# brendel-group/cl-ica

Hardware: AMD Instinct MI355X
Metric: training steps/sec (B=6144, n=10 MLP) (higher is better)
Workload: dtype f32 via f16x2 split (3 fp16 MFMA products of scaled two-piece operands, fp32 accumulate)

## Files before the change

cl_ica_amd/csrc/linear.hip:

```cpp
#include "common.h"
#include <string.h>
#include "wgrad_shared.h"
#include "split16.h"
#include "adam_math.h"
#include <stdlib.h>
#include <algorithm>

namespace clica {
bool skinny_fwd(const float* X, int64_t ldx, const float* W, int64_t ldw, const float* bias, float* Y, int64_t ldy,
                int64_t M, int64_t N, int64_t K, int leaky, float slope, hipStream_t st);
bool skinny_dgrad(const float* dY, int64_t lddy, const float* W, int64_t ldw, const float* Xact, int64_t ldxa, float slope,
                  float* dX, int64_t lddx, int64_t M, int64_t N, int64_t K, hipStream_t st);

namespace conv16 {
void launch_slab_sum(const float* slab1, int n1, float* out1, const float* slab2, int n2, float* out2, int splits, int accumulate, hipStream_t st);
}
namespace gemm {

typedef float f32x16 __attribute__((ext_vector_type(16)));

constexpr int BK = 32;
constexpr int RED_THREADS = 256;

enum Epi { EPI_BIAS_ACT = 0, EPI_DACT = 1, EPI_SLAB = 2 };
// ... 1045 lines not shown
        float* dst = G.dW[q] + i * G.lddw[q] + j;
        t.x = G.accumulate ? (*dst + t.x) : t.x;
        *dst = t.x;
        if (with_adam) adam_apply1(A, s_c, dst, t.x);
      }
    }
  } else {
    reduce_units<false>(G.dbslab[q], G.splits[q], M, (int64_t)(b - G.dw_blocks[q]) * 64, red, t, e);
    float* db = G.db[q];
    if (w == 0 && e < M) {
      t.x = G.accumulate ? (db[e] + t.x) : t.x;
      db[e] = t.x;
      if (with_adam) adam_apply1(A, s_c, db + e, t.x);
    }
  }
}

static void launch_slab_reduce(const float* slab, const float* dbslab, int splits, int64_t M, int64_t N, float* dW, int64_t lddw,
                               float* db, int accumulate, hipStream_t st) {
  const int64_t total = M * N;
  const bool v4 = (N % 4 == 0) && (lddw % 4 == 0) && ((reinterpret_cast<uintptr_t>(dW) & 15) == 0);
  const int dw_blocks = (int)ceil_div(v4 ? total / 4 : total, 64);
  const int db_blocks = db ? (int)ceil_div(M, 64) : 0;
  if (v4)
    hipLaunchKernelGGL(slab_reduce_k<true>, dim3((unsigned)(dw_blocks + db_blocks)), dim3(RED_THREADS), 0, st, slab, splits, M, N, dW, lddw,
                       dbslab, db, accumulate, dw_blocks);
  else
    hipLaunchKernelGGL(slab_reduce_k<false>, dim3((unsigned)(dw_blocks + db_blocks)), dim3(RED_THREADS), 0, st, slab, splits, M, N, dW, lddw,
                       dbslab, db, accumulate, dw_blocks);
}

static bool aligned16(const void* p) { return (reinterpret_cast<uintptr_t>(p) & 15) == 0; }

struct Cfg { int bm, bn, wm, wn; };
constexpr Cfg kCfgs[] = {
    {192, 128, 2, 4},
    {128, 128, 2, 4},
    {64, 128, 2, 2},
    {128, 128, 2, 2},
    {192, 64, 2, 2},
    {96, 128, 1, 4},
};
constexpr int kNumCfgs = sizeof(kCfgs) / sizeof(kCfgs[0]);

template <int BM, int BN, int WM, int WN, int STAGES, bool A_CONTIG, bool B_CONTIG, int EPI>
static int launch_cfg(const Args& g, int splits, hipStream_t st, const char* who) {
  constexpr int THREADS = 64 * WM * WN;
  const bool vec = aligned16(g.A) && aligned16(g.B) && (g.lda % 4 == 0) && (g.ldb % 4 == 0) &&
                   (A_CONTIG ? (g.Kc % 4 == 0) : (g.M % 4 == 0)) && (B_CONTIG ? (g.Kc % 4 == 0) : (g.N % 4 == 0));
  dim3 grid((unsigned)ceil_div(g.N, BN), (unsigned)ceil_div(g.M, BM), (unsigned)splits), block(THREADS);
  constexpr size_t lds = STAGES * (Tile<BM, A_CONTIG, THREADS>::LDS_FLOATS + Tile<BN, B_CONTIG, THREADS>::LDS_FLOATS) * sizeof(float);
  if (vec) {
    auto k = gemm_k<BM, BN, WM, WN, STAGES, A_CONTIG, B_CONTIG, EPI, true>;
    static bool once = ((void)hipFuncSetAttribute(reinterpret_cast<const void*>(k), hipFuncAttributeMaxDynamicSharedMemorySize, (int)lds), true);
    (void)once;
    hipLaunchKernelGGL(k, grid, block, lds, st, g);
  } else {
    auto k = gemm_k<BM, BN, WM, WN, STAGES, A_CONTIG, B_CONTIG, EPI, false>;
    static bool once = ((void)hipFuncSetAttribute(reinterpret_cast<const void*>(k), hipFuncAttributeMaxDynamicSharedMemorySize, (int)lds), true);
    (void)once;
    hipLaunchKernelGGL(k, grid, block, lds, st, g);
  }
  return launch_status(who);
}

template <bool A_CONTIG, bool B_CONTIG, int EPI>
static int launch(int cfg, const Args& g, int splits, hipStream_t st, const char* who) {
  switch (cfg) {
    case 0: return launch_cfg<192, 128, 2, 4, 3, A_CONTIG, B_CONTIG, EPI>(g, splits, st, who);
    case 1: return launch_cfg<128, 128, 2, 4, 3, A_CONTIG, B_CONTIG, EPI>(g, splits, st, who);
    case 2: return launch_cfg<64, 128, 2, 2, 2, A_CONTIG, B_CONTIG, EPI>(g, splits, st, who);
    case 4: return launch_cfg<192, 64, 2, 2, 2, A_CONTIG, B_CONTIG, EPI>(g, splits, st, who);
    case 5: return launch_cfg<96, 128, 1, 4, 2, A_CONTIG, B_CONTIG, EPI>(g, splits, st, who);
    default: return launch_cfg<128, 128, 2, 2, 2, A_CONTIG, B_CONTIG, EPI>(g, splits, st, who);
  }
}

struct Tuning { int cfg_fwd, cfg_dgrad, cfg_wgrad; bool skinny; };
static Tuning& tuning() { static Tuning t{-1, -1, -1, true}; return t; }
static bool use_skinny() { return tuning().skinny; }

static int cfg_fwd(int64_t N) {
  const int e = tuning().cfg_fwd;
  return (e >= 0 && e < kNumCfgs) ? e : ((N > 128) ? 5 : 2);
}
static int cfg_dgrad() {
  const int e = tuning().cfg_dgrad;
  return (e >= 0 && e < kNumCfgs) ? e : 2;
}

struct WgradPlan { int cfg, splits; int64_t k_per_split; };
static WgradPlan plan_wgrad(int64_t M , int64_t N , int64_t Kc) {
  WgradPlan p;
  p.cfg = (M > 128 && N > 128) ? 1 : 2;
  const int e = tuning().cfg_wgrad;
  if (e >= 0 && e < kNumCfgs) p.cfg = e;
  const Cfg c = kCfgs[p.cfg];
  const int64_t tiles = ceil_div(M, c.bm) * ceil_div(N, c.bn);
  int64_t want = kNumCU / tiles; if (want < 1) want = 1;
  const int64_t max_s = ceil_div(Kc, (int64_t)BK * 4);
  if (want > max_s) want = max_s;
  if (want < 1) want = 1;
  p.k_per_split = ceil_div(ceil_div(Kc, want), (int64_t)BK) * BK;
  p.splits = (int)ceil_div(Kc, p.k_per_split);
  return p;
}

struct GroupPlan { int splits; int64_t k_per_split; int tiles; int tiny_splits; int64_t tiny_kps; int n_tiny; };
constexpr int GBM = 128, GBN = 128;
static int group_kind(int32_t N, int32_t K) {
  if (tiny_eligible(N, K, TINY_THREADS)) return 2;
  if (N % 4 != 0 || K % 4 != 0) return 0;
  if (N > 128 || K > 128) return N >= K ? 3 : 4;
  return 1;
}
static void group_tile(int kind, int* bm, int* bn) {
  *bm = kind == 3 ? 256 : 128; *bn = kind == 4 ? 256 : 128;
}
static GroupPlan plan_wgrad_group(int64_t Mrows, int n, const int32_t* N, const int32_t* K) {
  GroupPlan p{};
  for (int l = 0; l < n; ++l) {
    const int kind = group_kind(N[l], K[l]);
    if (kind == 2) { ++p.n_tiny; continue; }
    int bm, bn; group_tile(kind, &bm, &bn);
    p.tiles += (int)(ceil_div(N[l], bm) * ceil_div(K[l], bn));
  }
  const int64_t max_s = std::max<int64_t>(1, std::min<int64_t>(64, ceil_div(Mrows, (int64_t)BK * 4)));
  double best = 1e300;
  p.splits = 1; p.k_per_split = ceil_div(Mrows, (int64_t)BK) * BK;
  for (int64_t s = 1; s <= max_s && p.tiles > 0; ++s) {
    const int64_t kps = ceil_div(ceil_div(Mrows, s), (int64_t)BK) * BK;
    const int64_t sp = ceil_div(Mrows, kps);
    const int64_t rounds = ceil_div((int64_t)p.tiles * sp, kNumCU);
    const double cost = (double)rounds * (kps + 32.0) + 8.0 * sp;
    if (cost < best) { best = cost; p.splits = (int)sp; p.k_per_split = kps; }
  }
  if (p.n_tiny > 0) wgrad_tiny_plan(Mrows, p.n_tiny, &p.tiny_splits, &p.tiny_kps);
  return p;
}
static bool group_is_tiny(const GroupPlan& p, int32_t N, int32_t K) { return p.n_tiny > 0 && group_kind(N, K) == 2; }
static size_t group_ws_layout(const GroupPlan& p, int n, const int32_t* N, const int32_t* K, size_t* slab_off, size_t* db_off) {
  size_t off = 0;
  for (int l = 0; l < n; ++l) {
    const size_t sp = group_is_tiny(p, N[l], K[l]) ? p.tiny_splits : p.splits;
    if (slab_off) slab_off[l] = off;
    off += align_up(sp * N[l] * K[l] * sizeof(float), 256);
    if (db_off) db_off[l] = off;
    off += align_up(sp * N[l] * sizeof(float), 256);
  }
  return off;
}


bool wgrad_tiny_shape(int32_t N, int32_t K) { return group_kind(N, K) == 2; }
void wgrad_tiny_plan(int64_t Mrows, int n_tiny, int* splits, int64_t* k_per_split) {
  int64_t ts = std::max<int64_t>(1, kNumCU / std::max(1, n_tiny));
  const int64_t cap = std::max<int64_t>(1, Mrows / (2 * TINY_ROWS));
  if (ts > cap) ts = cap;
  *k_per_split = ceil_div(ceil_div(Mrows, ts), (int64_t)TINY_ROWS) * TINY_ROWS;
  *splits = (int)ceil_div(Mrows, *k_per_split);
}
int launch_wgrad_tiny(const TinyArgs& T, int splits, hipStream_t st) {
  constexpr size_t tiny_lds = (size_t)(TINY_ROWS * TINY_MAX_LG + TINY_ROWS * TINY_MAX_S) * sizeof(float) + 1024;
  static bool once_t = ((void)hipFuncSetAttribute(reinterpret_cast<const void*>(wgrad_tiny_k), hipFuncAttributeMaxDynamicSharedMemorySize, (int)tiny_lds), true);
  (void)once_t;
  hipLaunchKernelGGL(wgrad_tiny_k, dim3((unsigned)splits, (unsigned)T.n), dim3(TINY_THREADS), tiny_lds, st, T);
  return launch_status("clica_mlp_wgrad(tiny)");
}
int launch_slab_reduce_group(const ReduceGroupArgs& R, int blocks, hipStream_t st) {
  const int front = (R.adam.p && R.adam.s16_state) ? s16::kS16UpdateBlocks : 0;
  hipLaunchKernelGGL(slab_reduce_group_k, dim3((unsigned)(blocks + front)), dim3(RED_THREADS), 0, st, R);
  return launch_status("clica_mlp_wgrad(reduce)");
}
int slab_reduce_entry(ReduceGroupArgs& R, int l, int first_block, int sp, const float* slab, const float* dbslab,
                      float* dW, int64_t lddw, float* db, int32_t N, int32_t K) {
  const bool v4 = (K % 4 == 0) && (lddw % 4 == 0) && aligned16(dW);
  R.vec4[l] = v4 ? 1 : 0; R.splits[l] = sp;
  R.dw_blocks[l] = (int)ceil_div(v4 ? (int64_t)N * K / 4 : (int64_t)N * K, reduce_flat(sp, v4) ? RED_THREADS : 64);
  R.first[l] = first_block;
  R.slab[l] = slab; R.dbslab[l] = dbslab; R.dW[l] = dW; R.db[l] = db;
  R.M[l] = N; R.N[l] = K; R.lddw[l] = lddw;
  return R.dw_blocks[l] + (db ? (int)ceil_div(N, 64) : 0);
}

}
}

using namespace clica;
using namespace clica::gemm;

extern "C" int clica_mlp_wgrad_workspace_bytes(int64_t M, int32_t n_layers, const int32_t* N, const int32_t* K, size_t* bytes) {
  CLICA_CHECK_ARG(bytes && N && K && M > 0 && n_layers >= 1 && n_layers <= MAXG, "clica_mlp_wgrad_workspace_bytes: bad argument");
  for (int l = 0; l < n_layers; ++l) CLICA_CHECK_ARG(N[l] >= 1 && K[l] >= 1, "clica_mlp_wgrad_workspace_bytes: layer %d: bad size", l);
  *bytes = group_ws_layout(plan_wgrad_group(M, n_layers, N, K), n_layers, N, K, nullptr, nullptr);
  return CLICA_OK;
}

extern "C" int clica_mlp_wgrad(int64_t M, int32_t n_layers, const float* const* dZ, const int64_t* lddz,
                               const float* const* X, const int64_t* ldx, float* const* dW, const int64_t* lddw,
                               float* const* db, const int32_t* N, const int32_t* K, int32_t accumulate,
                               void* workspace, size_t workspace_bytes, clica_stream_t stream) {
  CLICA_CHECK_ARG(dZ && lddz && X && ldx && dW && lddw && db && N && K && workspace && M > 0, "clica_mlp_wgrad: NULL pointer / empty batch");
  CLICA_CHECK_ARG(n_layers >= 1 && n_layers <= MAXG, "clica_mlp_wgrad: %d layers (1..%d supported)", n_layers, MAXG);
  for (int l = 0; l < n_layers; ++l) {
    CLICA_CHECK_ARG(dZ[l] && X[l] && dW[l] && N[l] >= 1 && K[l] >= 1, "clica_mlp_wgrad: layer %d: bad argument", l);
    CLICA_CHECK_ARG(lddz[l] >= N[l] && ldx[l] >= K[l] && lddw[l] >= K[l], "clica_mlp_wgrad: layer %d: leading dimension too small", l);
  }
  const GroupPlan p = plan_wgrad_group(M, n_layers, N, K);
  size_t slab_off[MAXG], db_off[MAXG];
  const size_t need = group_ws_layout(p, n_layers, N, K, slab_off, db_off);
  if (need > workspace_bytes) { set_error("clica_mlp_wgrad: workspace %zu < %zu", workspace_bytes, need); return CLICA_E_WORKSPACE; }
  hipStream_t st = as_stream(stream);
  GroupArgs G{};
  ReduceGroupArgs R{};
  TinyArgs T{};
  R.n = n_layers; R.accumulate = accumulate ? 1 : 0;
  int item = 0, rblock = 0, ng = 0;
  for (int l = 0; l < n_layers; ++l) {
    const bool tiny = group_is_tiny(p, N[l], K[l]);
    const int sp = tiny ? p.tiny_splits : p.splits;
    float* slab = (float*)((char*)workspace + slab_off[l]);
    float* dbslab = (float*)((char*)workspace + db_off[l]);
    Args g{};
    g.A = dZ[l]; g.lda = lddz[l]; g.B = X[l]; g.ldb = ldx[l]; g.C = slab; g.ldc = K[l]; g.M = N[l]; g.N = K[l]; g.Kc = M;
    g.k_per_split = tiny ? p.tiny_kps : p.k_per_split; g.dbias_slab = db[l] ? dbslab : nullptr;
    if (tiny) {
      T.p[T.n++] = g;
    } else {
      G.p[ng] = g;
      int kind = group_kind(N[l], K[l]);
      int bm, bn; group_tile(kind, &bm, &bn);
      if (!(aligned16(g.A) && aligned16(g.B) && g.lda % 4 == 0 && g.ldb % 4 == 0)) kind = (bm == 128 && bn == 128) ? 0 : -1;
      CLICA_CHECK_ARG(kind >= 0, "clica_mlp_wgrad: layer %d: operands of a %d x %d layer must be 16-byte aligned with leading "
                      "dimensions that are multiples of 4", l, N[l], K[l]);
      G.gx[ng] = (int)ceil_div(K[l], bn); G.gy[ng] = (int)ceil_div(N[l], bm);
      G.vec[ng] = kind;
      G.first[ng] = item; item += G.gx[ng] * G.gy[ng] * sp;
      ++ng;
    }
    rblock += slab_reduce_entry(R, l, rblock, sp, slab, dbslab, dW[l], lddw[l], db[l], N[l], K[l]);
  }
  G.n = ng; G.first[ng] = G.total = item; R.first[n_layers] = rblock;
  if (T.n > 0) {
    int rct = launch_wgrad_tiny(T, p.tiny_splits, st);
    if (rct) return rct;
  }
  if (ng > 0) {
    constexpr int WM = 2, WN = 4, STAGES = 3, THREADS = 64 * WM * WN;
    constexpr size_t lds1 = DMA_STAGES * (Tile<GBM, false, THREADS>::LDS_FLOATS + Tile<GBN, false, THREADS>::LDS_FLOATS) * sizeof(float);
    constexpr size_t lds = lds1 > kBody2LdsBytes ? lds1 : kBody2LdsBytes;
    auto k = wgrad_group_k<GBM, GBN, WM, WN, STAGES>;
    static bool once = ((void)hipFuncSetAttribute(reinterpret_cast<const void*>(k), hipFuncAttributeMaxDynamicSharedMemorySize, (int)lds), true);
    (void)once;
    hipLaunchKernelGGL(k, dim3((unsigned)item), dim3(THREADS), lds, st, G);
    int rc = launch_status("clica_mlp_wgrad");
    if (rc) return rc;
  }
  return launch_slab_reduce_group(R, rblock, st);
}

extern "C" int clica_linear_fwd(const float* X, int64_t ldx, const float* W, int64_t ldw, const float* bias,
                                float* Y, int64_t ldy, int64_t M, int64_t N, int64_t K,
                                int32_t leaky, float slope, clica_stream_t stream) {
  CLICA_CHECK_ARG(X && W && Y, "clica_linear_fwd: NULL pointer");
  CLICA_CHECK_ARG(M > 0 && N > 0 && K > 0, "clica_linear_fwd: M=%lld N=%lld K=%lld must be positive", (long long)M, (long long)N, (long long)K);
  CLICA_CHECK_ARG(ldx >= K && ldw >= K && ldy >= N, "clica_linear_fwd: leading dimension too small");
  if (use_skinny() && skinny_fwd(X, ldx, W, ldw, bias, Y, ldy, M, N, K, leaky, slope, as_stream(stream)))
    return launch_status("clica_linear_fwd(skinny)");
  Args g{}; g.A = X; g.lda = ldx; g.B = W; g.ldb = ldw; g.C = Y; g.ldc = ldy; g.M = M; g.N = N; g.Kc = K;
  g.bias = bias; g.slope = slope; g.leaky = leaky;
  const int cfg = cfg_fwd(N);
  return launch<true, true, EPI_BIAS_ACT>(cfg, g, 1, as_stream(stream), "clica_linear_fwd");
}

extern "C" int clica_linear_dgrad(const float* dY, int64_t lddy, const float* W, int64_t ldw,
                                  const float* Xact, int64_t ldxa, float slope,
                                  float* dX, int64_t lddx, int64_t M, int64_t N, int64_t K,
                                  clica_stream_t stream) {
  CLICA_CHECK_ARG(dY && W && dX, "clica_linear_dgrad: NULL pointer");
  CLICA_CHECK_ARG(M > 0 && N > 0 && K > 0, "clica_linear_dgrad: sizes must be positive");
  CLICA_CHECK_ARG(lddy >= N && ldw >= K && lddx >= K && (!Xact || ldxa >= K), "clica_linear_dgrad: leading dimension too small");
  if (use_skinny() && skinny_dgrad(dY, lddy, W, ldw, Xact, ldxa, slope, dX, lddx, M, N, K, as_stream(stream)))
    return launch_status("clica_linear_dgrad(skinny)");
  Args g{}; g.A = dY; g.lda = lddy; g.B = W; g.ldb = ldw; g.C = dX; g.ldc = lddx; g.M = M; g.N = K; g.Kc = N;
  g.xact = Xact; g.ldxa = ldxa; g.slope = slope;
  const int cfg = cfg_dgrad();
  return launch<true, false, EPI_DACT>(cfg, g, 1, as_stream(stream), "clica_linear_dgrad");
}

extern "C" int clica_linear_plan(int32_t op, int64_t M, int64_t N, int64_t K, int32_t* tile_m, int32_t* tile_n,
                                 int32_t* waves, int32_t* splits) {
  CLICA_CHECK_ARG(op >= 0 && op <= 2 && M > 0 && N > 0 && K > 0, "clica_linear_plan: bad argument");
  int cfg, sp = 1;
  if (op == 0) cfg = cfg_fwd(N);
  else if (op == 1) cfg = cfg_dgrad();
  else { const WgradPlan p = plan_wgrad(N, K, M); cfg = p.cfg; sp = p.splits; }
  if (tile_m) *tile_m = kCfgs[cfg].bm;
  if (tile_n) *tile_n = kCfgs[cfg].bn;
  if (waves) *waves = kCfgs[cfg].wm * kCfgs[cfg].wn;
  if (splits) *splits = sp;
  return CLICA_OK;
}

namespace clica { namespace lp { void set_dot_mfma(int on); void set_fused_finalize(int on); } }
namespace clica { namespace wsplit { void set_epi_specialised(int on); } }
extern "C" int clica_set_tuning(const char* key, int32_t value) {
  CLICA_CHECK_ARG(key != nullptr, "clica_set_tuning: key is NULL");
  gemm::Tuning& t = gemm::tuning();
  if (!strcmp(key, "skinny")) t.skinny = value != 0;
  else if (!strcmp(key, "gemm_cfg_fwd")) t.cfg_fwd = value;
  else if (!strcmp(key, "gemm_cfg_dgrad")) t.cfg_dgrad = value;
  else if (!strcmp(key, "gemm_cfg_wgrad")) t.cfg_wgrad = value;
  else if (!strcmp(key, "dot_mfma")) clica::lp::set_dot_mfma(value);
  else if (!strcmp(key, "gemm16_epilogue")) clica::wsplit::set_epi_specialised(value);
  else if (!strcmp(key, "lp_fused_finalize")) clica::lp::set_fused_finalize(value);
  else if (!strcmp(key, "reset")) { t = gemm::Tuning{-1, -1, -1, true}; clica::lp::set_dot_mfma(1); clica::wsplit::set_epi_specialised(1); clica::lp::set_fused_finalize(1); }
  else { set_error("clica_set_tuning: unknown key '%s'", key); return CLICA_E_INVALID; }
  return CLICA_OK;
}

extern "C" int clica_linear_wgrad_workspace_bytes(int64_t M, int64_t N, int64_t K, size_t* bytes) {
  CLICA_CHECK_ARG(bytes && M > 0 && N > 0 && K > 0, "clica_linear_wgrad_workspace_bytes: bad argument");
  const int64_t max_s = ceil_div(M, (int64_t)BK * 4) < kNumCU ? ceil_div(M, (int64_t)BK * 4) : kNumCU;
  *bytes = align_up((size_t)max_s * N * K * sizeof(float), 256) + align_up((size_t)max_s * N * sizeof(float), 256);
  const WgradPlan p = plan_wgrad(N, K, M);
  const size_t exact = align_up((size_t)p.splits * N * K * sizeof(float), 256) + align_up((size_t)p.splits * N * sizeof(float), 256);
  if (tuning().cfg_wgrad < 0) *bytes = exact;
  return CLICA_OK;
}

extern "C" int clica_linear_wgrad(const float* dY, int64_t lddy, const float* X, int64_t ldx,
                                  float* dW, int64_t lddw, float* db, int64_t M, int64_t N, int64_t K,
                                  int32_t accumulate, void* workspace, size_t workspace_bytes,
                                  clica_stream_t stream) {
  CLICA_CHECK_ARG(dY && X && dW && workspace, "clica_linear_wgrad: NULL pointer");
  CLICA_CHECK_ARG(M > 0 && N > 0 && K > 0, "clica_linear_wgrad: sizes must be positive");
  CLICA_CHECK_ARG(lddy >= N && ldx >= K && lddw >= K, "clica_linear_wgrad: leading dimension too small");
  hipStream_t st = as_stream(stream);
  const WgradPlan p = plan_wgrad(N, K, M);
  const size_t slab_bytes = align_up((size_t)p.splits * N * K * sizeof(float), 256);
  const size_t need = slab_bytes + align_up((size_t)p.splits * N * sizeof(float), 256);
  if (need > workspace_bytes) { set_error("clica_linear_wgrad: workspace %zu < %zu", workspace_bytes, need); return CLICA_E_WORKSPACE; }
  float* slab = (float*)workspace;
  float* dbslab = (float*)((char*)workspace + slab_bytes);
  Args g{}; g.A = dY; g.lda = lddy; g.B = X; g.ldb = ldx; g.C = slab; g.ldc = K; g.M = N; g.N = K; g.Kc = M;
  g.k_per_split = p.k_per_split;
  g.dbias_slab = db ? dbslab : nullptr;
  int rc;
  const bool vec = aligned16(g.A) && aligned16(g.B) && g.lda % 4 == 0 && g.ldb % 4 == 0 && N % 4 == 0 && K % 4 == 0;
  if (vec && p.cfg == 1) {
    GroupArgs G{};
    G.n = 1; G.p[0] = g; G.vec[0] = 1;
    G.gx[0] = (int)ceil_div(K, GBN); G.gy[0] = (int)ceil_div(N, GBM);
    G.first[0] = 0; G.first[1] = G.total = G.gx[0] * G.gy[0] * p.splits;
    constexpr int WM = 2, WN = 4, STAGES = 3, THREADS = 64 * WM * WN;
    constexpr size_t lds = DMA_STAGES * (Tile<GBM, false, THREADS>::LDS_FLOATS + Tile<GBN, false, THREADS>::LDS_FLOATS) * sizeof(float);
    constexpr size_t lds_max = lds > kBody2LdsBytes ? lds : kBody2LdsBytes;
    auto k = wgrad_group_k<GBM, GBN, WM, WN, STAGES>;
    static bool once = ((void)hipFuncSetAttribute(reinterpret_cast<const void*>(k), hipFuncAttributeMaxDynamicSharedMemorySize, (int)lds_max), true);
    (void)once;
    hipLaunchKernelGGL(k, dim3((unsigned)G.total), dim3(THREADS), lds, st, G);
    rc = launch_status("clica_linear_wgrad");
  } else {
    rc = launch<false, false, EPI_SLAB>(p.cfg, g, p.splits, st, "clica_linear_wgrad");
  }
  if (rc) return rc;
  launch_slab_reduce(slab, dbslab, p.splits, N, K, dW, lddw, db, accumulate ? 1 : 0, st);
  return launch_status("clica_linear_wgrad(reduce)");
}

namespace clica {
namespace gemm {

template <int BM, int BN, int WM, int WN, int STAGES, bool A_CONTIG, bool B_CONTIG, int EPI>
__global__ __launch_bounds__(64 * WM * WN) void conv_gemm_k(Args g, ConvX cx) {
  const int gx = gridDim.x, gxy = gx * gridDim.y;
  const int id = xcd_contiguous(blockIdx.z * gxy + blockIdx.y * gx + blockIdx.x, gxy * gridDim.z);
  const int bz = id / gxy, rem = id - bz * gxy, by = rem / gx;
  gemm_body<BM, BN, WM, WN, STAGES, A_CONTIG, B_CONTIG, EPI, true, true>(g, rem - by * gx, by, bz, cx);
}

template <int BM, int BN, int WM, int WN, int STAGES, bool A_CONTIG, bool B_CONTIG, int EPI>
static int launch_conv(const Args& g, const ConvX& cx, int splits, hipStream_t st, const char* who) {
  constexpr int THREADS = 64 * WM * WN;
  dim3 grid((unsigned)ceil_div(g.N, BN), (unsigned)ceil_div(g.M, BM), (unsigned)splits), block(THREADS);
  constexpr size_t lds = STAGES * (Tile<BM, A_CONTIG, THREADS>::LDS_FLOATS + Tile<BN, B_CONTIG, THREADS>::LDS_FLOATS) * sizeof(float);
  auto k = conv_gemm_k<BM, BN, WM, WN, STAGES, A_CONTIG, B_CONTIG, EPI>;
  static bool once = ((void)hipFuncSetAttribute(reinterpret_cast<const void*>(k), hipFuncAttributeMaxDynamicSharedMemorySize, (int)lds), true);
  (void)once;
  hipLaunchKernelGGL(k, grid, block, lds, st, g, cx);
  return launch_status(who);
}

static int conv_fwd_launch(const float* A, int64_t lda, int64_t seg, int64_t jump, const float* Wg, const float* bias, int64_t rows,
                           int32_t K, int32_t Cout, int32_t hs, int32_t ws, int32_t ho, int32_t wo, int32_t relu, int32_t scatter,
                           float* out, uint32_t* gate_bits, hipStream_t st, const char* who, int compact = 0) {
  const int ghs = hs, gws = ws;
  const bool fast_ok = K % BK == 0 && lda % 4 == 0 && jump % 4 == 0 && seg % 4 == 0 && jump < (1 << 30);
  if (compact && fast_ok && scatter) { rows = rows / ((int64_t)hs * ws) * ((int64_t)ho * wo); hs = ho; ws = wo; } else { compact = 0; }
  if (scatter == 2 && !compact) { set_error("%s: scatter = 2 needs a contraction of whole k-tiles", who); return CLICA_E_INVALID; }
  Args g{}; g.A = A; g.lda = lda; g.B = Wg; g.ldb = K; g.C = out; g.ldc = Cout; g.M = rows; g.N = Cout; g.Kc = K;
  g.bias = bias; g.leaky = relu ? 1 : 0; g.slope = 0.f;
  ConvX cx{}; cx.a_seg = seg; cx.a_jump = jump; cx.mode = scatter == 2 ? 3 : (scatter ? 1 : 0);
  cx.hs = hs; cx.ws = ws; cx.ho = ho; cx.wo = wo; cx.dhs = ho / 2 + 1; cx.dws = wo / 2 + 1; cx.c = Cout;
  cx.inv_pix = 1.f / (float)(hs * ws); cx.inv_ws = 1.f / (float)ws;
  cx.gate_out = gate_bits;
  cx.fast = fast_ok ? 1 : 0;
  cx.compact = compact; cx.ghs = ghs; cx.gws = gws;
  if (gate_bits && !(scatter == 1 && Cout % 32 == 0)) { set_error("%s: gate bits need the scattering epilogue and Cout %% 32 == 0", who); return CLICA_E_INVALID; }
  if (scatter && rows >= (1 << 24)) { set_error("%s: %lld rows (the scattering epilogue handles < 2^24)", who, (long long)rows); return CLICA_E_INVALID; }
  if (Cout > 64 && rows <= 8192) return launch_conv<64, 64, 2, 2, 2, true, true, EPI_BIAS_ACT>(g, cx, 1, st, who);
  if (Cout <= 32) return launch_conv<128, 32, 4, 1, 2, true, true, EPI_BIAS_ACT>(g, cx, 1, st, who);
  if (Cout <= 64) return launch_conv<128, 64, 2, 2, 2, true, true, EPI_BIAS_ACT>(g, cx, 1, st, who);
  return launch_conv<64, 128, 2, 2, 2, true, true, EPI_BIAS_ACT>(g, cx, 1, st, who);
}

constexpr int DG_ROWS = 256;
__global__ __launch_bounds__(512) void conv_dgrad32_stream_k(const float* __restrict__ A0 , const float* __restrict__ Wd,
                                                             int64_t rows, float* __restrict__ dst, ConvX cx) {
  extern __shared__ __attribute__((aligned(16))) float sB[];
  const int ws = cx.ws;
  const int lane = threadIdx.x & 63, wave = threadIdx.x >> 6, h = lane >> 5, l31 = lane & 31;
  for (int u = threadIdx.x; u < 128 * 32; u += 512) reinterpret_cast<float4*>(sB)[u] = reinterpret_cast<const float4*>(Wd)[u];
  __syncthreads();
  const int64_t ntiles = (rows + DG_ROWS - 1) / DG_ROWS;
  const int64_t last = rows + ws;
  for (int64_t tile = blockIdx.x; tile < ntiles; tile += gridDim.x) {
    const int64_t r0 = tile * DG_ROWS;
    const int64_t rbase = r0 + wave * 32 + l31;
    auto lda = [&](int st) {
      const int64_t gr = min(rbase + (st >> 3) * ws + ((st & 7) >> 2), last);
      return *reinterpret_cast<const float4*>(A0 + gr * 32 + 8 * (st & 3) + 4 * h);
    };
    f32x16 acc[4];
#pragma unroll
    for (int j = 0; j < 4; ++j)
#pragma unroll
      for (int r = 0; r < 16; ++r) acc[j][r] = 0.f;
    float4 aq[3];
    aq[0] = lda(0); aq[1] = lda(1);
    float b4[2][4][4];
    auto bfr = [&](int buf, int st) {
#pragma unroll
      for (int j = 0; j < 4; ++j)
#pragma unroll
        for (int t = 0; t < 4; ++t) b4[buf][j][t] = sB[(8 * st + 4 * h + t) * 128 + j * 32 + l31];
    };
    bfr(0, 0);
#pragma unroll
    for (int st = 0; st < 16; ++st) {
      if (st + 2 < 16) aq[(st + 2) % 3] = lda(st + 2);
      if (st + 1 < 16) bfr((st + 1) & 1, st + 1);
      __builtin_amdgcn_sched_barrier(0);
      const float4 av = aq[st % 3];
      const float a4[4] = {av.x, av.y, av.z, av.w};
#pragma unroll
      for (int t = 0; t < 4; ++t)
#pragma unroll
        for (int j = 0; j < 4; ++j) acc[j] = __builtin_amdgcn_mfma_f32_32x32x2f32(a4[t], b4[st & 1][j][t], acc[j], 0, 0, 0);
      __builtin_amdgcn_sched_barrier(0);
    }
#pragma unroll
    for (int r = 0; r < 16; ++r) {
      const int64_t row = r0 + wave * 32 + (r & 3) + 8 * (r >> 2) + 4 * h;
      if (row >= rows) continue;
      int img, y, x;
      conv_row_to_pixel(cx, row, img, y, x);
#pragma unroll
      for (int j = 0; j < 4; ++j) {
        const int yy = 2 * y + (j >> 1) - 1, xx = 2 * x + (j & 1) - 1;
        if (yy < 0 || xx < 0 || yy >= cx.dho || xx >= cx.dwo) continue;
        const int64_t pix = ((int64_t)img * cx.dhs + yy) * cx.dws + xx;
        const unsigned word = cx.gate_in[pix];
        dst[pix * 32 + l31] = ((word >> l31) & 1u) ? acc[j][r] : 0.f;
      }
    }
  }
}

struct ConvWgradPlan { int bm, splits; int64_t k_per_split; };
static ConvWgradPlan plan_conv_wgrad(int64_t rows, int32_t Cout, int32_t K) {
  ConvWgradPlan p;
  p.bm = Cout <= 32 ? 32 : 64;
  const int64_t tiles = ceil_div(Cout, p.bm) * ceil_div(K, 128);
  int64_t want = std::max<int64_t>(1, 3 * kNumCU / tiles);
  want = std::min<int64_t>(want, std::max<int64_t>(1, rows / (8 * BK)));
  p.k_per_split = ceil_div(ceil_div(rows, want), (int64_t)BK) * BK;
  p.splits = (int)ceil_div(rows, p.k_per_split);
  return p;
}

__global__ __launch_bounds__(256) void conv_im2col_k4s2_k(const float* __restrict__ x, unsigned pixels, int C, int H, int W,
                                                           float* __restrict__ patches) {
  const unsigned t = blockIdx.x * 256u + threadIdx.x;
  const unsigned pixel = t >> 4, tap = t & 15u;
  if (pixel >= pixels) return;
  const unsigned Wo = W / 2, Ho = H / 2;
  const unsigned prow = pixel / Wo, ox = pixel - prow * Wo, img = prow / Ho, oy = prow - img * Ho;
  const int y = 2 * (int)oy + (int)(tap >> 2) - 1, xx = 2 * (int)ox + (int)(tap & 3u) - 1;
  const bool in = y >= 0 && y < H && xx >= 0 && xx < W;
  const float* src = x + ((int64_t)img * C * H + y) * W + xx;
  float* dst = patches + ((int64_t)pixel * 16 + tap) * C;
  for (int c = 0; c < C; ++c) dst[c] = in ? src[(int64_t)c * H * W] : 0.f;
}

__global__ __launch_bounds__(256) void conv_im2col_k4s2_c1_k(const float* __restrict__ x, unsigned pixels, int H, int W, float* __restrict__ patches) {
  const unsigned t = blockIdx.x * 256u + threadIdx.x;
  const unsigned pixel = t >> 2, ky = t & 3u;
  if (pixel >= pixels) return;
  const unsigned Wo = W / 2, Ho = H / 2;
  const unsigned prow = pixel / Wo, ox = pixel - prow * Wo, img = prow / Ho, oy = prow - img * Ho;
  const int y = 2 * (int)oy + (int)ky - 1, x0 = 2 * (int)ox - 1;
  const bool rin = y >= 0 && y < H;
  const float* rowp = x + ((int64_t)img * H + (rin ? y : 0)) * W;
  const bool i0 = rin && x0 >= 0, i3 = rin && x0 + 3 < W;
  const float v0 = rowp[i0 ? x0 : 0], v1 = rowp[x0 + 1], v2 = rowp[x0 + 2], v3 = rowp[i3 ? x0 + 3 : 0];
  *reinterpret_cast<float4*>(patches + (int64_t)pixel * 16 + 4 * ky) = make_float4(i0 ? v0 : 0.f, rin ? v1 : 0.f, rin ? v2 : 0.f, i3 ? v3 : 0.f);
}

__global__ __launch_bounds__(256) void conv_wgrad_patches_k(const float* __restrict__ dO, const float* __restrict__ P, int64_t rows,
                                                             int Cout, int K, int64_t rows_per_block, float* __restrict__ slab,
                                                             float* __restrict__ dbslab) {
  extern __shared__ float red[];
  const int ncg = Cout / 4, gsz = ncg * (K / 4), G = 256 / gsz;
  const int g = threadIdx.x / gsz, u = threadIdx.x - g * gsz, cg = u % ncg, kg = u / ncg;
  const int64_t r0 = (int64_t)blockIdx.x * rows_per_block, r1 = min(rows, r0 + rows_per_block);
  float acc[4][4] = {};
  float4 bsum = make_float4(0.f, 0.f, 0.f, 0.f);
  if (g < G) {
#pragma unroll 4
    for (int64_t r = r0 + g; r < r1; r += G) {
      const float4 d = *reinterpret_cast<const float4*>(dO + r * Cout + 4 * cg);
      const float4 p = *reinterpret_cast<const float4*>(P + r * K + 4 * kg);
      const float dv[4] = {d.x, d.y, d.z, d.w}, pv[4] = {p.x, p.y, p.z, p.w};
#pragma unroll
      for (int i = 0; i < 4; ++i)
#pragma unroll
        for (int j = 0; j < 4; ++j) acc[i][j] = fmaf(dv[i], pv[j], acc[i][j]);
      bsum.x += d.x; bsum.y += d.y; bsum.z += d.z; bsum.w += d.w;
    }
    float* mine = red + (size_t)g * (Cout * K + Cout);
#pragma unroll
    for (int i = 0; i < 4; ++i)
#pragma unroll
      for (int j = 0; j < 4; ++j) mine[(4 * cg + i) * K + 4 * kg + j] = acc[i][j];
    if (kg == 0) { mine[Cout * K + 4 * cg] = bsum.x; mine[Cout * K + 4 * cg + 1] = bsum.y; mine[Cout * K + 4 * cg + 2] = bsum.z; mine[Cout * K + 4 * cg + 3] = bsum.w; }
  }
  __syncthreads();
  const int per = Cout * K + Cout;
  for (int e = threadIdx.x; e < per; e += 256) {
    float v = 0.f;
    for (int gg = 0; gg < G; ++gg) v += red[(size_t)gg * per + e];
    if (e < Cout * K) slab[(int64_t)blockIdx.x * Cout * K + e] = v;
    else if (dbslab) dbslab[(int64_t)blockIdx.x * Cout + (e - Cout * K)] = v;
  }
}

template <int K>
__global__ __launch_bounds__(256) void conv_fwd_patches_valu_k(const float* __restrict__ P, const float* __restrict__ Wg,
                                                                const float* __restrict__ bias, unsigned pixels, int Cout, int ho, int wo,
                                                                int relu, float* __restrict__ out, unsigned* __restrict__ gate_out,
                                                                unsigned* __restrict__ amax_slots) {
  const int groups = Cout / 8;
  float amax = 0.f;
  const int cg = threadIdx.x % groups;
  const int half = Cout / 2;
  auto chan = [&](int c) { return c < 4 ? 4 * cg + c : half + 4 * cg + (c - 4); };
  float w[8][K], b[8];
#pragma unroll
  for (int c = 0; c < 8; ++c) {
    b[c] = bias ? bias[chan(c)] : 0.f;
#pragma unroll
    for (int k = 0; k < K; ++k) w[c][k] = Wg[chan(c) * K + k];
  }
  const unsigned per_block = 256 / groups, stride = gridDim.x * per_block;
  const int dhs = ho / 2 + 1, dws = wo / 2 + 1;
  float4 nxt[K / 4];
  const unsigned first = blockIdx.x * per_block + threadIdx.x / groups;
  if (first < pixels) {
#pragma unroll
    for (int k = 0; k < K; k += 4) nxt[k / 4] = *reinterpret_cast<const float4*>(P + (int64_t)first * K + k);
  }
  for (unsigned pixel = first; pixel < pixels; pixel += stride) {
    float a[K];
#pragma unroll
    for (int k = 0; k < K; k += 4) { a[k] = nxt[k / 4].x; a[k + 1] = nxt[k / 4].y; a[k + 2] = nxt[k / 4].z; a[k + 3] = nxt[k / 4].w; }
    if (pixel + stride < pixels) {
#pragma unroll
      for (int k = 0; k < K; k += 4) nxt[k / 4] = *reinterpret_cast<const float4*>(P + (int64_t)(pixel + stride) * K + k);
    }
    float o[8];
#pragma unroll
    for (int c = 0; c < 8; ++c) {
      float acc = 0.f;
#pragma unroll
      for (int k = 0; k < K; ++k) acc = fmaf(a[k], w[c][k], acc);
      acc += b[c];
      o[c] = (relu && !(acc > 0.f)) ? 0.f : acc;
      amax = fmaxf(amax, fabsf(o[c]));
    }
    const unsigned prow = pixel / (unsigned)wo, x = pixel - prow * (unsigned)wo, img = prow / (unsigned)ho, y = prow - img * (unsigned)ho;
    const unsigned Y = (y + 1) >> 1, X = (x + 1) >> 1, qq = ((y + 1) & 1) * 2 + ((x + 1) & 1);
    float* dst = out + (((int64_t)img * dhs + Y) * dws + X) * (4 * Cout) + qq * Cout + 4 * cg;
    *reinterpret_cast<float4*>(dst) = make_float4(o[0], o[1], o[2], o[3]);
    *reinterpret_cast<float4*>(dst + half) = make_float4(o[4], o[5], o[6], o[7]);
    if (gate_out) {
      unsigned bits = 0;
#pragma unroll
      for (int c = 0; c < 8; ++c) bits |= (o[c] > 0.f ? 1u : 0u) << chan(c);
      bits |= __shfl_xor(bits, 1);
      bits |= __shfl_xor(bits, 2);
      if (cg == 0) gate_out[pixel] = bits;
    }
  }
  if (amax_slots) {
#pragma unroll
    for (int off = 32; off > 0; off >>= 1) amax = fmaxf(amax, __shfl_xor(amax, off, 64));
    if ((threadIdx.x & 63) == 0) {
      amax = (amax <= 3.0e38f) ? amax : 3.4e38f;
// ... 555 lines not shown
```

cl_ica_amd/csrc/lp_finalize.h:

```cpp
#pragma once
#include "lp_kernels.h"

namespace clica {
namespace lp {

__device__ __forceinline__ float pos_sum(const float* a, const float* b, int n, const Params& q, bool frac) {
  float s = 0.f;
  for (int k = 0; k < n; ++k) {
    float d = a[k] - b[k];
    float t;
    if (frac) t = fexp2(q.p * flog2(fabsf(d) + 1e-12f));
    else if (q.p == 2.f) t = d * d;
    else if (q.p == 1.f) t = fabsf(d);
    else if (q.p == 3.f) t = fabsf(d) * d * d;
    else t = fabsf(d) > 0.f ? fexp2(q.p * flog2(fabsf(d))) : 0.f;
    s += t;
  }
  return s;
}

struct Means {
  float* blocksums;
};

__device__ __forceinline__ void reduce_means(float v0, float v1, float v2, const Means& M, const int blk, const bool coherent = false) {
  __shared__ float red[3][THREADS / 64];
  float v[3] = {v0, v1, v2};
#pragma unroll
  for (int a = 0; a < 3; ++a) {
#pragma unroll
    for (int off = 32; off > 0; off >>= 1) v[a] += __shfl_down(v[a], off, 64);
  }
  const int wave = threadIdx.x >> 6, lane = threadIdx.x & 63;
  if (lane == 0) { red[0][wave] = v[0]; red[1][wave] = v[1]; red[2][wave] = v[2]; }
  __syncthreads();
  if (threadIdx.x < 3) {
    float t = 0.f;
    for (int w = 0; w < THREADS / 64; ++w) t += red[threadIdx.x][w];
    if (coherent) __hip_atomic_store(&M.blocksums[blk * 3 + threadIdx.x], t, __ATOMIC_RELAXED, __HIP_MEMORY_SCOPE_AGENT);
    else M.blocksums[blk * 3 + threadIdx.x] = t;
  }
}


constexpr int FIN_ROWS = 64;
struct TrainOut { float* statL; float* statC; float* dz1; int64_t ldd1; float* dz2; int64_t ldd2; };

__device__ __forceinline__ void coef_row(
    const int64_t i, const int64_t rows, const float* a , const float* b ,
    const Params& q, float tau, float alpha, int compat, int frac, int dot, const float L2,
    const float* __restrict__ g_mean, const float* __restrict__ g_item,
    const float* __restrict__ g_pos, const float* __restrict__ g_neg,
    float* __restrict__ statL, float* __restrict__ statC,
    float* __restrict__ dz1, int64_t ldd1, float* __restrict__ dz2, int64_t ldd2, float* statC_value = nullptr) {
  const float inv_rows = 1.f / (float)rows;
  const float gi = (g_mean ? g_mean[0] : 1.f) * inv_rows + (g_item ? g_item[i] : 0.f);
  const float A = 2.f * alpha * gi + (g_pos ? g_pos[0] * inv_rows : 0.f);
  const float C = 2.f * (1.f - alpha) * gi + (g_neg ? g_neg[0] * inv_rows : 0.f);
  statL[i] = L2;
  const float sc = q.xs * C / tau;
  statC[i] = sc;
  if (statC_value) *statC_value = sc;
  if (!dz1 && !dz2) return;
  if (dot) {
    float pos = 0.f;
    if (q.posdot) pos = q.posdot[i];
    else for (int k = 0; k < q.n; ++k) pos += a[k] * b[k];
    const float dpos = -A / tau + (C / tau) * fexp2(pos * q.kscale - L2);
    if (q.dpos) { q.dpos[i] = dpos; return; }
    for (int k = 0; k < q.n; ++k) {
      if (dz1) dz1[i * ldd1 + k] = dpos * b[k];
      if (dz2) dz2[i * ldd2 + k] = dpos * a[k];
    }
    return;
  }
  const float sp_ = pos_sum(a, b, q.n, q, frac != 0);
  const float pos = q.pow ? sp_ : root_of<true>(sp_, q);
  float cpos = A / tau;
  if (compat) cpos -= (C / tau) * fexp2(-pos * q.kscale - L2);
  cpos *= q.pow ? q.p : droot_of<true>(sp_, q);
  for (int k = 0; k < q.n; ++k) {
    const float d = a[k] - b[k];
    float dt;
    if (frac) {
      const float v = fexp2((q.p - 1.f) * flog2(fabsf(d) + 1e-12f));
      dt = d > 0.f ? v : (d < 0.f ? -v : 0.f);
    } else if (q.p == 2.f) dt = d;
    else if (q.p == 1.f) dt = (d > 0.f ? 1.f : 0.f) - (d < 0.f ? 1.f : 0.f);
    else if (q.p == 3.f) dt = d * fabsf(d);
    else {
      const float ad = fabsf(d);
      const float v = ad > 0.f ? fexp2((q.p - 1.f) * flog2(ad)) : 0.f;
      dt = d < 0.f ? -v : v;
    }
    const float g = cpos * dt;
    if (dz1) dz1[i * ldd1 + k] = g;
    if (dz2) dz2[i * ldd2 + k] = -g;
  }
}


struct FinScratch { float* sm; float* ss; float* zr0; float* zr1; int zmaxn; float* ush; };
template <bool COHERENT = false>
__device__ __forceinline__ void finalize_rows(
    const int blk, const float2* __restrict__ part, const int nsplit, const int64_t rows,
    const float* __restrict__ z1, int64_t ld1, const float* __restrict__ z2, int64_t ld2,
    const Params& q, float tau, float alpha, int compat, int frac, int dot, float log_b3,
    float* __restrict__ loss_i, float* __restrict__ pos_i, float* __restrict__ lse_i, const TrainOut& T, const FinScratch& S,
    float& v_loss, float& v_pos, float& v_lse) {
  const int lane_row = threadIdx.x & (FIN_ROWS - 1), grp = threadIdx.x / FIN_ROWS;
  const int64_t i = (int64_t)blk * FIN_ROWS + lane_row;
  const bool staged = q.n <= S.zmaxn;
  if (staged) {
    const int64_t r0 = (int64_t)blk * FIN_ROWS;
    const int cnt = (int)min((int64_t)FIN_ROWS, rows - r0) * q.n;
    for (int idx = threadIdx.x; idx < cnt; idx += THREADS) {
      const int r = idx / q.n, k = idx - r * q.n;
      S.zr0[idx] = z1[(r0 + r) * ld1 + k];
      S.zr1[idx] = z2[(r0 + r) * ld2 + k];
    }
  }
  float m = -1e30f, s = 0.f;
  if (i < rows) {
    constexpr int G = THREADS / FIN_ROWS;
    for (int sp0 = grp; sp0 < nsplit; sp0 += 4 * G) {
      float2 ps[4];
#pragma unroll
      for (int u = 0; u < 4; ++u) {
        const int sp = sp0 + u * G;
        if (!(sp < nsplit)) ps[u] = make_float2(-1e30f, 0.f);
        else if (COHERENT)
          ps[u] = __builtin_bit_cast(float2, __hip_atomic_load(reinterpret_cast<const unsigned long long*>(part + (int64_t)sp * rows + i),
                                                                __ATOMIC_RELAXED, __HIP_MEMORY_SCOPE_AGENT));
        else ps[u] = part[(int64_t)sp * rows + i];
      }
#pragma unroll
      for (int u = 0; u < 4; ++u) {
        const float mn = fmaxf(m, ps[u].x);
        s = s * fexp2(m - mn) + ps[u].y * fexp2(ps[u].x - mn);
        m = mn;
      }
    }
  }
  S.sm[grp * FIN_ROWS + lane_row] = m; S.ss[grp * FIN_ROWS + lane_row] = s;
  __syncthreads();
  v_loss = 0.f; v_pos = 0.f; v_lse = 0.f;
  if (grp == 0 && i < rows) {
#pragma unroll
    for (int w = 1; w < THREADS / FIN_ROWS; ++w) {
      const float pm = S.sm[w * FIN_ROWS + lane_row], psum = S.ss[w * FIN_ROWS + lane_row];
      const float mn = fmaxf(m, pm);
      s = s * fexp2(m - mn) + psum * fexp2(pm - mn);
      m = mn;
    }
    float pos, xp;
    const float* ra = staged ? &S.zr0[lane_row * q.n] : z1 + i * ld1;
    const float* rb = staged ? &S.zr1[lane_row * q.n] : z2 + i * ld2;
    if (dot) {
      pos = 0.f;
      if (q.posdot) pos = q.posdot[i];
      else for (int k = 0; k < q.n; ++k) pos += ra[k] * rb[k];
      xp = pos * q.kscale;
      pos = -pos;
    } else {
      const float sp_ = pos_sum(ra, rb, q.n, q, frac != 0);
      pos = q.pow ? sp_ : root_of<true>(sp_, q);
      xp = -pos * q.kscale;
    }
    if (compat) {
      const float mn = fmaxf(m, xp);
      s = s * fexp2(m - mn) + fexp2(xp - mn);
      m = mn;
    }
    const float L2 = m + flog2(s);
    const float lse_raw = L2 * kLn2;
    const float lse = compat ? lse_raw : lse_raw - log_b3;
    const float lp = pos / tau;
    const float li = 2.f * (alpha * lp + (1.f - alpha) * lse);
    loss_i[i] = li; pos_i[i] = lp; lse_i[i] = L2;
    float sc_i = 0.f;
    if (T.statL)
      coef_row(i, rows, ra, rb, q, tau, alpha, compat, frac, dot, L2, nullptr, nullptr, nullptr, nullptr, T.statL, T.statC,
               T.dz1, T.ldd1, T.dz2, T.ldd2, &sc_i);
    v_loss = li; v_pos = lp; v_lse = lse;
    if (S.ush) S.ush[lane_row] = sc_i * fexp2(-L2);
  } else if (S.ush && grp == 0) {
    S.ush[lane_row] = 0.f;
  }
}

struct FinArgs {
  const float* z2; int64_t ld2; float tau, alpha; int compat; float log_b3;
  float* loss_i; float* pos_i; float* lse_i; Means M; TrainOut T; int* arrive;
  float* means; float inv_count;
};
template <int NP, int PK, int R, bool ROOT, int NQ, bool ZMAX>
__global__ __launch_bounds__(THREADS, fwd_min_waves(NP, false)) void fwd_partial_fin_k(
    const float* __restrict__ own, int64_t ldo, int64_t n_own,
    const float* __restrict__ str, int64_t lds, int64_t n_str,
    Params q, float2* __restrict__ part, int chunk, FinArgs F) {
  static_assert(HALF * R == FIN_ROWS && NP <= 16, "an owner tile of the sweep = one finalize block; z rows staged in the tile buffers");
  float* scratch = nullptr;
  fwd_partial_body<NP, PK, R, ROOT, false, NQ, ZMAX>(own, ldo, n_own, str, lds, n_str, q, part, nullptr, chunk, blockIdx.x, blockIdx.y, &scratch);
  __shared__ float sm[THREADS / FIN_ROWS][FIN_ROWS], ss[THREADS / FIN_ROWS][FIN_ROWS];
  __shared__ int s_last;
  __builtin_amdgcn_s_waitcnt(0x0F70);
  __syncthreads();
  if (threadIdx.x == 0) {
    const int prev = __hip_atomic_fetch_add(&F.arrive[blockIdx.x], 1, __ATOMIC_RELAXED, __HIP_MEMORY_SCOPE_AGENT);
    s_last = prev == (int)gridDim.y - 1;
    if (s_last) __hip_atomic_store(&F.arrive[blockIdx.x], 0, __ATOMIC_RELAXED, __HIP_MEMORY_SCOPE_AGENT);
  }
  __syncthreads();
  if (!s_last) return;
  float v_loss, v_pos, v_lse;
  constexpr int ZMAXN = 2 * tile_rows(NP) * NP / (2 * FIN_ROWS);
  static_assert(ZMAXN >= NP, "tile buffers too small for the z rows");
  finalize_rows<true>((int)blockIdx.x, part, (int)gridDim.y, n_own, own, ldo, F.z2, F.ld2, q, F.tau, F.alpha, F.compat, 0, 0, F.log_b3,
                F.loss_i, F.pos_i, F.lse_i, F.T, FinScratch{&sm[0][0], &ss[0][0], scratch, scratch + FIN_ROWS * ZMAXN, ZMAXN, nullptr},
                v_loss, v_pos, v_lse);
  reduce_means(v_loss, v_pos, v_lse, F.M, (int)blockIdx.x, F.means != nullptr);
  if (!F.means) return;
  __builtin_amdgcn_s_waitcnt(0x0F70);
  __syncthreads();
  if (threadIdx.x == 0) {
    const int prev = __hip_atomic_fetch_add(&F.arrive[gridDim.x], 1, __ATOMIC_RELAXED, __HIP_MEMORY_SCOPE_AGENT);
    s_last = prev == (int)gridDim.x - 1;
    if (s_last) __hip_atomic_store(&F.arrive[gridDim.x], 0, __ATOMIC_RELAXED, __HIP_MEMORY_SCOPE_AGENT);
  }
  __syncthreads();
  if (!s_last || threadIdx.x >= 64) return;
  float v[3] = {0.f, 0.f, 0.f};
  for (int b = threadIdx.x; b < (int)gridDim.x; b += 64) {
#pragma unroll
    for (int c = 0; c < 3; ++c) v[c] += __hip_atomic_load(&F.M.blocksums[b * 3 + c], __ATOMIC_RELAXED, __HIP_MEMORY_SCOPE_AGENT);
  }
#pragma unroll
  for (int a = 0; a < 3; ++a) {
#pragma unroll
    for (int off = 32; off > 0; off >>= 1) v[a] += __shfl_down(v[a], off, 64);
  }
  if (threadIdx.x == 0) { F.means[0] = v[0] * F.inv_count; F.means[1] = v[1] * F.inv_count; F.means[2] = v[2] * F.inv_count; }
}

#define CLICA_LP_DECLARE_FIN(PKV)                                                                          \
  bool launch_fwd_partial_fin_pk##PKV(const Plan& P, const float* own, int64_t ldo, int64_t n_own,        \
                                      const float* str, int64_t lds, int64_t n_str, const Params& q,      \
                                      float2* part, const FinArgs& F, hipStream_t st);
CLICA_LP_DECLARE_FIN(0) CLICA_LP_DECLARE_FIN(1) CLICA_LP_DECLARE_FIN(2) CLICA_LP_DECLARE_FIN(3) CLICA_LP_DECLARE_FIN(4)

}
}
```

cl_ica_amd/csrc/lp_kernels.h:

```cpp
#pragma once
#include "common.h"
#include <math.h>
#include <stdlib.h>
#include <type_traits>

namespace clica {
namespace lp {

constexpr int THREADS = 256;
constexpr int WAVES = THREADS / 64;
constexpr int HALF = 32;
constexpr int PARTS = 2 * WAVES;
constexpr int JB = 4;
#ifndef CLICA_LP_JBW
#define CLICA_LP_JBW 2
#endif
constexpr int jb_fwd(int np) { return np <= 16 ? 4 : 2; }
constexpr int JBW = CLICA_LP_JBW;
#ifndef CLICA_LP_TS16
#define CLICA_LP_TS16 128
#endif
#ifndef CLICA_LP_TS40
#define CLICA_LP_TS40 128
#endif
constexpr int tile_rows(int np) { return np <= 16 ? CLICA_LP_TS16 : (np <= 40 ? CLICA_LP_TS40 : 64); }

struct Params {
  float p;
  float inv_p;
  float kscale;
  float sgn;
  float eps;
  float xs;
  int pow;
  int n;
  int train = 0;
  float pre = 1.f;
  float gfold = 1.f;
  const float* posdot = nullptr;
  float* dpos = nullptr;
};

typedef float f32x2 __attribute__((ext_vector_type(2)));

__device__ __forceinline__ float fexp2(float x) { return __builtin_amdgcn_exp2f(x); }
__device__ __forceinline__ float flog2(float x) { return __builtin_amdgcn_logf(x); }

constexpr int PK_DOT = 4;

__device__ __forceinline__ float add_abs(float acc, float d) {
  float r;
  asm("v_add_f32_e64 %0, %1, |%2|" : "=v"(r) : "v"(acc), "v"(d));
  return r;
}

template <int PK>
__device__ __forceinline__ void accum2(f32x2& acc, f32x2 o, f32x2 s, const Params& q, int k) {
  if constexpr (PK == PK_DOT) {
    acc = __builtin_elementwise_fma(o, s, acc);
  } else if constexpr (PK == 2) {
    const f32x2 d = o - s;
    acc = __builtin_elementwise_fma(d, d, acc);
  } else if constexpr (PK == 1) {
    const f32x2 d = o - s;
    acc.x = add_abs(acc.x, d.x); acc.y = add_abs(acc.y, d.y);
  } else if constexpr (PK == 3) {
    const f32x2 d = o - s, t = d * d;
    acc.x = fmaf(fabsf(d.x), t.x, acc.x); acc.y = fmaf(fabsf(d.y), t.y, acc.y);
  } else {
    if (k < q.n) { const float a = fabsf(q.sgn * (o.x - s.x) + q.eps); acc.x += a > 0.f ? fexp2(q.p * flog2(a)) : 0.f; }
    if (k + 1 < q.n) { const float a = fabsf(q.sgn * (o.y - s.y) + q.eps); acc.y += a > 0.f ? fexp2(q.p * flog2(a)) : 0.f; }
  }
}
template <int PK>
__device__ __forceinline__ void gaccum2(f32x2& g, float coef, f32x2 o, f32x2 s, const Params& q, int k) {
  const f32x2 c2 = {coef, coef};
  if constexpr (PK == PK_DOT) {
    g = __builtin_elementwise_fma(c2, s, g);
  } else if constexpr (PK == 2) {
    g = __builtin_elementwise_fma(c2, o - s, g);
  } else if constexpr (PK == 1) {
    const f32x2 d = o - s;
    const f32x2 big = {0x1p126f, 0x1p126f};
    f32x2 t = d * big;
    t.x = __builtin_amdgcn_fmed3f(t.x, -1.f, 1.f); t.y = __builtin_amdgcn_fmed3f(t.y, -1.f, 1.f);
    g = __builtin_elementwise_fma(c2, t, g);
  } else if constexpr (PK == 3) {
    const f32x2 d = o - s;
    const f32x2 t = {d.x * fabsf(d.x), d.y * fabsf(d.y)};
    g = __builtin_elementwise_fma(c2, t, g);
  } else {
    if (k < q.n) {
      const float e = q.sgn * (o.x - s.x) + q.eps, a = fabsf(e);
      const float v = a > 0.f ? fexp2((q.p - 1.f) * flog2(a)) : 0.f;
      g.x += coef * (e < 0.f ? -v : v);
    }
    if (k + 1 < q.n) {
      const float e = q.sgn * (o.y - s.y) + q.eps, a = fabsf(e);
      const float v = a > 0.f ? fexp2((q.p - 1.f) * flog2(a)) : 0.f;
      g.y += coef * (e < 0.f ? -v : v);
    }
  }
}
template <bool ROOT>
__device__ __forceinline__ float root_of(float s, const Params& q) {
  if constexpr (!ROOT) return s;
  if (q.p == 2.f) return sqrtf(s);
  if (q.p == 1.f) return s;
  return s > 0.f ? fexp2(q.inv_p * flog2(s)) : 0.f;
}
template <bool ROOT>
__device__ __forceinline__ float droot_of(float s, const Params& q) {
  if constexpr (!ROOT) return q.p;
  if (q.p == 1.f) return 1.f;
  return s > 0.f ? fexp2((q.inv_p - 1.f) * flog2(s)) : 0.f;
}

template <int NP>
struct Stager {
  static constexpr int TS = tile_rows(NP);
  static constexpr int ITERS = TS * NP / THREADS;
  static_assert((TS * NP) % THREADS == 0, "tile must divide over the workgroup");
  float v[ITERS];
  __device__ __forceinline__ void load(const float* __restrict__ str, int64_t lds, int64_t j0, int cnt, int n, float pre = 1.f) {
#pragma unroll
    for (int it = 0; it < ITERS; ++it) {
      const int idx = threadIdx.x + it * THREADS;
      const int row = idx / NP, k = idx - row * NP;
      const bool ok = row < cnt && k < n;
      const float x = str[ok ? (j0 + row) * lds + k : 0];
      v[it] = ok ? x * pre : 0.f;
    }
  }
  __device__ __forceinline__ void store(float* tile) const {
#pragma unroll
    for (int it = 0; it < ITERS; ++it) tile[threadIdx.x + it * THREADS] = v[it];
  }
};

template <int NP, int R>
__device__ __forceinline__ void load_owners(f32x2 (&o)[R][NP / 2], const float* __restrict__ own, int64_t ldo,
                                            int64_t own0, int64_t n_own, int n, float pre = 1.f) {
  const int li = threadIdx.x & (HALF - 1);
#pragma unroll
  for (int r = 0; r < R; ++r) {
    const int64_t i = own0 + (int64_t)r * HALF + li;
    const bool ok = i < n_own;
#pragma unroll
    for (int k2 = 0; k2 < NP / 2; ++k2) {
      const bool a = ok && 2 * k2 < n, b = ok && 2 * k2 + 1 < n;
      const float x = own[a ? i * ldo + 2 * k2 : 0], y = own[b ? i * ldo + 2 * k2 + 1 : 0];
      o[r][k2].x = a ? x * pre : 0.f; o[r][k2].y = b ? y * pre : 0.f;
    }
  }
}

template <int NP, int PK, int NQ = NP / 2, int JBT = JB>
__device__ __forceinline__ void dist_group(const f32x2 (&o)[NP / 2], const float* tile, int jj, const Params& q,
                                           float (&acc)[JBT]) {
  f32x2 a2[JBT];
#pragma unroll
  for (int c = 0; c < JBT; ++c) a2[c] = (f32x2){0.f, 0.f};
#pragma unroll
  for (int k4 = 0; k4 < NP / 4; ++k4) {
#pragma unroll
    for (int c = 0; c < JBT; ++c) {
      const float4 sv = *reinterpret_cast<const float4*>(&tile[(jj + c) * NP + 4 * k4]);
      if (2 * k4 < NQ) accum2<PK>(a2[c], o[2 * k4], (f32x2){sv.x, sv.y}, q, 4 * k4);
      if (2 * k4 + 1 < NQ) accum2<PK>(a2[c], o[2 * k4 + 1], (f32x2){sv.z, sv.w}, q, 4 * k4 + 2);
    }
  }
#pragma unroll
  for (int c = 0; c < JBT; ++c) acc[c] = a2[c].x + a2[c].y;
}

template <int NP, int PK, int NQ = NP / 2, int JBT = JB>
__device__ __forceinline__ void dist_group_keep(const f32x2 (&o)[NP / 2], const float* tile, int jj, float (&acc)[JBT], f32x2 (&d)[JBT][NQ]) {
  static_assert(PK >= 1 && PK <= 3, "difference-based pair kinds");
  f32x2 a2[JBT];
#pragma unroll
  for (int c = 0; c < JBT; ++c) a2[c] = (f32x2){0.f, 0.f};
#pragma unroll
  for (int k4 = 0; k4 < NP / 4; ++k4) {
#pragma unroll
    for (int c = 0; c < JBT; ++c) {
      const float4 sv = *reinterpret_cast<const float4*>(&tile[(jj + c) * NP + 4 * k4]);
#pragma unroll
      for (int h2 = 0; h2 < 2; ++h2) {
        const int k2 = 2 * k4 + h2;
        if (k2 < NQ) {
          const f32x2 dd = o[k2] - (h2 ? (f32x2){sv.z, sv.w} : (f32x2){sv.x, sv.y});
          d[c][k2] = dd;
          if constexpr (PK == 2) a2[c] = __builtin_elementwise_fma(dd, dd, a2[c]);
          else if constexpr (PK == 1) { a2[c].x = add_abs(a2[c].x, dd.x); a2[c].y = add_abs(a2[c].y, dd.y); }
          else { const f32x2 t = dd * dd; a2[c].x = fmaf(fabsf(dd.x), t.x, a2[c].x); a2[c].y = fmaf(fabsf(dd.y), t.y, a2[c].y); }
        }
      }
    }
  }
#pragma unroll
  for (int c = 0; c < JBT; ++c) acc[c] = a2[c].x + a2[c].y;
}
template <int PK>
__device__ __forceinline__ void gaccum2_d(f32x2& g, float coef, f32x2 d) {
  const f32x2 c2 = {coef, coef};
  if constexpr (PK == 2) {
    g = __builtin_elementwise_fma(c2, d, g);
  } else if constexpr (PK == 1) {
    const f32x2 big = {0x1p126f, 0x1p126f};
    f32x2 t = d * big;
    t.x = __builtin_amdgcn_fmed3f(t.x, -1.f, 1.f); t.y = __builtin_amdgcn_fmed3f(t.y, -1.f, 1.f);
    g = __builtin_elementwise_fma(c2, t, g);
  } else {
    const f32x2 t = {d.x * fabsf(d.x), d.y * fabsf(d.y)};
    g = __builtin_elementwise_fma(c2, t, g);
  }
}

constexpr int fwd_min_waves(int np, bool rowgrad) { return rowgrad ? (np <= 16 ? 3 : 2) : (np <= 16 ? 4 : (np <= 24 ? 3 : 2)); }
constexpr int bwd_min_waves(int np) { return np <= 16 ? 3 : 2; }

template <int NP, int PK, int R, bool ROOT, bool ROWGRAD, int NQ = NP / 2, bool ZMAX = false>
__device__ __forceinline__ void fwd_partial_body(
    const float* __restrict__ own, int64_t ldo, int64_t n_own,
    const float* __restrict__ str, int64_t lds, int64_t n_str,
    const Params& q, float2* __restrict__ part, float* __restrict__ part_g, int chunk, const int bx, const int by,
    float** scratch_out = nullptr ) {
  constexpr int TS = tile_rows(NP), RPP = TS / PARTS, JBF = jb_fwd(NP);
  static_assert(RPP % JBF == 0, "partition rows must be whole JB groups");
  static_assert(WAVES * HALF * R * NP <= 2 * TS * NP, "the cross-wave merge reuses the tile buffers");
  __shared__ __attribute__((aligned(16))) float tiles[2][TS * NP];
  __shared__ float2 wred[WAVES][HALF * R];
  if (scratch_out) *scratch_out = &tiles[0][0];
  const int lane = threadIdx.x & 63, wave = threadIdx.x >> 6, li = lane & (HALF - 1), hf = lane >> 5;
  const int pq = wave * 2 + hf;
  const int64_t own0 = (int64_t)bx * (HALF * R);
  f32x2 o[R][NP / 2];
  f32x2 G[ROWGRAD ? R : 1][NP / 2];
  load_owners<NP, R>(o, own, ldo, own0, n_own, q.n, q.pre);
  float m[R], s[R];
  const float csgn = (PK == 0) ? q.sgn : 1.f;
#pragma unroll
  for (int r = 0; r < (ROWGRAD ? R : 1); ++r)
#pragma unroll
    for (int k2 = 0; k2 < NP / 2; ++k2) G[r][k2] = (f32x2){0.f, 0.f};
  static_assert(!(ZMAX && ROWGRAD), "the fixed-maximum forward is the training sweep (no row gradient)");
#pragma unroll
  for (int r = 0; r < R; ++r) { m[r] = ZMAX ? 0.f : -INFINITY; s[r] = 0.f; }
  const float xk = q.xs * q.kscale;

  const int64_t jb = (int64_t)by * chunk;
  const int64_t je = min(n_str, jb + (int64_t)chunk);
  Stager<NP> st;
  if (jb < je) {
    st.load(str, lds, jb, (int)min((int64_t)TS, je - jb), q.n, q.pre);
    st.store(tiles[0]);
  }
  __syncthreads();
  int cur = 0;
  for (int64_t j0 = jb; j0 < je; j0 += TS, cur ^= 1) {
    const int cnt = (int)min((int64_t)TS, je - j0);
    const bool more = j0 + TS < je;
    if (more) st.load(str, lds, j0 + TS, (int)min((int64_t)TS, je - j0 - TS), q.n, q.pre);
    const float* tile = tiles[cur] + pq * RPP * NP;
    const int cq = min(RPP, max(0, cnt - pq * RPP));
    auto sweep = [&](auto ragged_tag) {
    constexpr bool RAGGED = decltype(ragged_tag)::value;
    for (int jj = 0; jj < cq; jj += JBF) {
#pragma unroll
      for (int r = 0; r < R; ++r) {
        float acc[JBF];
        dist_group<NP, PK, NQ, JBF>(o[r], tile, jj, q, acc);
        if constexpr (ZMAX) {
          float add = 0.f;
#pragma unroll
          for (int c = 0; c < JBF; ++c) add += (RAGGED && jj + c >= cq) ? 0.f : fexp2(PK == 1 ? acc[c] * xk : -acc[c]);
          s[r] += add;
          continue;
        }
        float x[JBF];
#pragma unroll
        for (int c = 0; c < JBF; ++c) {
          x[c] = root_of<ROOT>(acc[c], q) * xk;
          if (RAGGED && jj + c >= cq) x[c] = -INFINITY;
        }
        float xm = x[0];
#pragma unroll
        for (int c = 1; c < JBF; ++c) xm = fmaxf(xm, x[c]);
        const float mn = fmaxf(xm, fmaxf(m[r], -1e30f));
        float add = 0.f, e[JBF];
#pragma unroll
        for (int c = 0; c < JBF; ++c) { e[c] = fexp2(x[c] - mn); add += e[c]; }
        const float resc = fexp2(m[r] - mn);
        s[r] = fmaf(s[r], resc, add);
        m[r] = mn;
        if (ROWGRAD) {
#pragma unroll
          for (int c = 0; c < JBF; ++c) e[c] *= droot_of<ROOT>(acc[c], q) * csgn;
          asm volatile("" ::: "memory");
          const f32x2 r2 = {resc, resc};
#pragma unroll
          for (int k4 = 0; k4 < NP / 4; ++k4) {
            G[r][2 * k4] *= r2; G[r][2 * k4 + 1] *= r2;
#pragma unroll
            for (int c = 0; c < JBF; ++c) {
              const float4 sv = *reinterpret_cast<const float4*>(&tile[(jj + c) * NP + 4 * k4]);
              if (2 * k4 < NQ) gaccum2<PK>(G[r][2 * k4], e[c], o[r][2 * k4], (f32x2){sv.x, sv.y}, q, 4 * k4);
              if (2 * k4 + 1 < NQ) gaccum2<PK>(G[r][2 * k4 + 1], e[c], o[r][2 * k4 + 1], (f32x2){sv.z, sv.w}, q, 4 * k4 + 2);
            }
          }
        }
      }
    }
    };
    if (cq == RPP) sweep(std::false_type{}); else sweep(std::true_type{});
    if (more) st.store(tiles[cur ^ 1]);
    __syncthreads();
  }
  float* gred = &tiles[0][0];
#pragma unroll
  for (int r = 0; r < R; ++r) {
    const float mo = __shfl_xor(m[r], HALF, 64), so = __shfl_xor(s[r], HALF, 64);
    const float mn = fmaxf(fmaxf(m[r], mo), -1e30f);
    const float fa = fexp2(m[r] - mn), fb = fexp2(mo - mn);
    const float s_lo = hf ? so : s[r], s_hi = hf ? s[r] : so, f_lo = hf ? fb : fa, f_hi = hf ? fa : fb;
    s[r] = fmaf(s_lo, f_lo, s_hi * f_hi);
    if (ROWGRAD) {
#pragma unroll
      for (int k2 = 0; k2 < NP / 2; ++k2) {
        const float gxo = __shfl_xor(G[r][k2].x, HALF, 64), gyo = __shfl_xor(G[r][k2].y, HALF, 64);
        const float gx_lo = hf ? gxo : G[r][k2].x, gx_hi = hf ? G[r][k2].x : gxo;
        const float gy_lo = hf ? gyo : G[r][k2].y, gy_hi = hf ? G[r][k2].y : gyo;
        G[r][k2].x = fmaf(gx_lo, f_lo, gx_hi * f_hi); G[r][k2].y = fmaf(gy_lo, f_lo, gy_hi * f_hi);
      }
    }
    m[r] = mn;
    if (hf == 0) {
      wred[wave][r * HALF + li] = make_float2(m[r], s[r]);
      if (ROWGRAD) {
        float4* dst = reinterpret_cast<float4*>(gred + ((size_t)wave * (HALF * R) + r * HALF + li) * NP);
#pragma unroll
        for (int k4 = 0; k4 < NP / 4; ++k4)
          dst[k4] = make_float4(G[r][2 * k4].x, G[r][2 * k4].y, G[r][2 * k4 + 1].x, G[r][2 * k4 + 1].y);
      }
    }
  }
  __syncthreads();
  if (threadIdx.x < HALF * R) {
    const int t = threadIdx.x;
    const int64_t i = own0 + t;
    float mm = -1e30f;
#pragma unroll
    for (int w = 0; w < WAVES; ++w) mm = fmaxf(mm, wred[w][t].x);
    float ss = 0.f, f[WAVES];
#pragma unroll
    for (int w = 0; w < WAVES; ++w) { f[w] = fexp2(wred[w][t].x - mm); ss = fmaf(wred[w][t].y, f[w], ss); }
    if (i < n_own) {
      if (scratch_out) {
        const float2 ms = make_float2(mm, ss);
        __hip_atomic_store(reinterpret_cast<unsigned long long*>(part + (int64_t)by * n_own + i), __builtin_bit_cast(unsigned long long, ms),
                           __ATOMIC_RELAXED, __HIP_MEMORY_SCOPE_AGENT);
      } else {
        part[(int64_t)by * n_own + i] = make_float2(mm, ss);
      }
      if (ROWGRAD) {
        float4* dst = reinterpret_cast<float4*>(part_g + ((int64_t)by * n_own + i) * NP);
#pragma unroll
        for (int k4 = 0; k4 < NP / 4; ++k4) {
          float4 a4 = make_float4(0.f, 0.f, 0.f, 0.f);
#pragma unroll
          for (int w = 0; w < WAVES; ++w) {
            const float4 g4 = *reinterpret_cast<const float4*>(gred + ((size_t)w * (HALF * R) + t) * NP + 4 * k4);
            a4.x = fmaf(g4.x, f[w], a4.x); a4.y = fmaf(g4.y, f[w], a4.y); a4.z = fmaf(g4.z, f[w], a4.z); a4.w = fmaf(g4.w, f[w], a4.w);
          }
          dst[k4] = a4;
        }
      }
    }
  }
}

template <int NP, int PK, int R, bool ROOT, bool ROWGRAD, int NQ = NP / 2, bool ZMAX = false>
__global__ __launch_bounds__(THREADS, fwd_min_waves(NP, ROWGRAD)) void fwd_partial_k(
    const float* __restrict__ own, int64_t ldo, int64_t n_own,
    const float* __restrict__ str, int64_t lds, int64_t n_str,
    Params q, float2* __restrict__ part, float* __restrict__ part_g, int chunk) {
  fwd_partial_body<NP, PK, R, ROOT, ROWGRAD, NQ, ZMAX>(own, ldo, n_own, str, lds, n_str, q, part, part_g, chunk, blockIdx.x, blockIdx.y);
}

template <int NP, int PK, int R, int STATS, bool ROOT, int NQ = NP / 2, bool FOLD = false>
__device__ __forceinline__ void bwd_pairs_body(
    const float* __restrict__ own, int64_t ldo, int64_t n_own,
    const float* __restrict__ str, int64_t lds, int64_t n_str,
    const Params& q, const float* __restrict__ statL, const float* __restrict__ statC,
    const float* __restrict__ strL, const float* __restrict__ strC,
    float* __restrict__ part, int chunk, const int bx, const int by) {
  constexpr bool OWNER_STATS = (STATS & 1) != 0, STREAM_STATS = (STATS & 2) != 0;
  constexpr int TS = tile_rows(NP), RPP = TS / PARTS;
  static_assert(WAVES * HALF * R * NP <= 2 * TS * NP, "the cross-wave merge reuses the tile buffers");
  __shared__ __attribute__((aligned(16))) float tiles[2][TS * NP];
  __shared__ float tLs[2][TS], tCs[2][TS];
  const int lane = threadIdx.x & 63, wave = threadIdx.x >> 6, li = lane & (HALF - 1), hf = lane >> 5;
  const int pq = wave * 2 + hf;
  const int64_t own0 = (int64_t)bx * (HALF * R);
  f32x2 o[R][NP / 2], g[R][NP / 2];
  load_owners<NP, R>(o, own, ldo, own0, n_own, q.n, q.pre);
  float oL[R], oC[R];
#pragma unroll
  for (int r = 0; r < R; ++r) {
    const int64_t i = own0 + (int64_t)r * HALF + li;
    oL[r] = 0.f; oC[r] = 0.f;
    if (OWNER_STATS && i < n_own) { oL[r] = statL[i]; oC[r] = statC[i]; }
    if (FOLD) oC[r] *= fexp2(-oL[r]) * q.gfold;
#pragma unroll
    for (int k2 = 0; k2 < NP / 2; ++k2) g[r][k2] = (f32x2){0.f, 0.f};
  }
  const float xk = q.xs * q.kscale;
  const float csgn = (PK == 0) ? q.sgn : 1.f;
  const int64_t jb = (int64_t)by * chunk;
  const int64_t je = min(n_str, jb + (int64_t)chunk);
  Stager<NP> st;
  float rl = 0.f, rc = 0.f;
  auto load_stats = [&](int64_t j0, int cnt) {
    if (STREAM_STATS && (int)threadIdx.x < TS) {
      const bool ok = (int)threadIdx.x < cnt;
      const float l = strL[ok ? j0 + threadIdx.x : 0], c = strC[ok ? j0 + threadIdx.x : 0];
      rl = ok ? l : 0.f;
      rc = ok ? c : 0.f;
    }
  };
  auto store_stats = [&](int b) {
    if (STREAM_STATS && (int)threadIdx.x < TS) { tLs[b][threadIdx.x] = rl; tCs[b][threadIdx.x] = FOLD ? rc * fexp2(-rl) * q.gfold : rc; }
  };
  if (jb < je) {
    const int c0 = (int)min((int64_t)TS, je - jb);
    st.load(str, lds, jb, c0, q.n, q.pre); load_stats(jb, c0);
    st.store(tiles[0]); store_stats(0);
  }
  __syncthreads();
  int cur = 0;
  for (int64_t j0 = jb; j0 < je; j0 += TS, cur ^= 1) {
    const int cnt = (int)min((int64_t)TS, je - j0);
    const bool more = j0 + TS < je;
    if (more) {
      const int c1 = (int)min((int64_t)TS, je - j0 - TS);
      st.load(str, lds, j0 + TS, c1, q.n, q.pre); load_stats(j0 + TS, c1);
    }
    const float* tile = tiles[cur] + pq * RPP * NP;
    const float* tL = tLs[cur] + pq * RPP;
    const float* tC = tCs[cur] + pq * RPP;
    const int cq = min(RPP, max(0, cnt - pq * RPP));
#ifndef CLICA_LP_KEEPD_WIDE
#define CLICA_LP_KEEPD_WIDE 1
#endif
    constexpr bool KEEPD = PK >= 1 && PK <= 3 && (NP <= 16 || (CLICA_LP_KEEPD_WIDE && NP <= 40));
    constexpr int JW = KEEPD ? 1 : JBW;
    for (int jj = 0; jj < cq; jj += JW) {
#pragma unroll
      for (int r = 0; r < R; ++r) {
        float acc[JW];
        f32x2 dk[JW][KEEPD ? NQ : 1];
        if constexpr (KEEPD) dist_group_keep<NP, PK, NQ, JW>(o[r], tile, jj, acc, dk);
        else dist_group<NP, PK, NQ, JW>(o[r], tile, jj, q, acc);
        float coef[JW];
#pragma unroll
        for (int c = 0; c < JW; ++c) {
          if constexpr (FOLD) {
            static_assert(!FOLD || (STATS == 3 && !ROOT), "folded coefficient: symmetric training sweep only");
            float cf = fexp2(PK == 1 ? acc[c] * xk : -acc[c]) * (oC[r] + tC[jj + c]);
            if (jj + c >= cq) cf = 0.f;
            coef[c] = cf;
            continue;
          }
          const float x = root_of<ROOT>(acc[c], q) * xk;
          float w = 0.f;
          if constexpr (FOLD) {
          } else {
            if (OWNER_STATS) w = oC[r] * fexp2(x - oL[r]);
            if (STREAM_STATS) w = fmaf(tC[jj + c], fexp2(x - tL[jj + c]), w);
          }
          float cf = w * droot_of<ROOT>(acc[c], q) * csgn;
          if (OWNER_STATS && jj + c >= cq) cf = 0.f;
          coef[c] = cf;
        }
        if constexpr (KEEPD) {
#pragma unroll
          for (int k2 = 0; k2 < NQ; ++k2)
#pragma unroll
            for (int c = 0; c < JW; ++c) gaccum2_d<PK>(g[r][k2], coef[c], dk[c][k2]);
        } else {
          asm volatile("" ::: "memory");
#pragma unroll
          for (int k4 = 0; k4 < NP / 4; ++k4) {
#pragma unroll
            for (int c = 0; c < JW; ++c) {
              const float4 sv = *reinterpret_cast<const float4*>(&tile[(jj + c) * NP + 4 * k4]);
              if (2 * k4 < NQ) gaccum2<PK>(g[r][2 * k4], coef[c], o[r][2 * k4], (f32x2){sv.x, sv.y}, q, 4 * k4);
              if (2 * k4 + 1 < NQ) gaccum2<PK>(g[r][2 * k4 + 1], coef[c], o[r][2 * k4 + 1], (f32x2){sv.z, sv.w}, q, 4 * k4 + 2);
            }
          }
        }
      }
    }
    if (more) { st.store(tiles[cur ^ 1]); store_stats(cur ^ 1); }
    __syncthreads();
  }
  float* gred = &tiles[0][0];
#pragma unroll
  for (int r = 0; r < R; ++r) {
#pragma unroll
    for (int k2 = 0; k2 < NP / 2; ++k2) {
      const float gxo = __shfl_xor(g[r][k2].x, HALF, 64), gyo = __shfl_xor(g[r][k2].y, HALF, 64);
      g[r][k2].x = hf ? gxo + g[r][k2].x : g[r][k2].x + gxo;
      g[r][k2].y = hf ? gyo + g[r][k2].y : g[r][k2].y + gyo;
    }
    if (hf == 0) {
      float4* dst = reinterpret_cast<float4*>(gred + ((size_t)wave * (HALF * R) + r * HALF + li) * NP);
#pragma unroll
      for (int k4 = 0; k4 < NP / 4; ++k4)
        dst[k4] = make_float4(g[r][2 * k4].x, g[r][2 * k4].y, g[r][2 * k4 + 1].x, g[r][2 * k4 + 1].y);
    }
  }
  __syncthreads();
  constexpr int Q4 = NP / 4;
  for (int u = threadIdx.x; u < HALF * R * Q4; u += THREADS) {
    const int t = u / Q4, k4 = u - t * Q4;
    const int64_t i = own0 + t;
    if (i >= n_own) continue;
    float4 a4 = *reinterpret_cast<const float4*>(gred + (size_t)t * NP + 4 * k4);
#pragma unroll
    for (int w = 1; w < WAVES; ++w) {
      const float4 g4 = *reinterpret_cast<const float4*>(gred + ((size_t)w * (HALF * R) + t) * NP + 4 * k4);
      a4.x += g4.x; a4.y += g4.y; a4.z += g4.z; a4.w += g4.w;
    }
    *reinterpret_cast<float4*>(part + ((int64_t)by * n_own + i) * NP + 4 * k4) = a4;
  }
}

template <int NP, int PK, int R, int STATS, bool ROOT, int NQ = NP / 2, bool FOLD = false>
__global__ __launch_bounds__(THREADS, bwd_min_waves(NP)) void bwd_pairs_k(
    const float* __restrict__ own, int64_t ldo, int64_t n_own,
    const float* __restrict__ str, int64_t lds, int64_t n_str,
    Params q, const float* __restrict__ statL, const float* __restrict__ statC,
    const float* __restrict__ strL, const float* __restrict__ strC,
    float* __restrict__ part, int chunk) {
  bwd_pairs_body<NP, PK, R, STATS, ROOT, NQ, FOLD>(own, ldo, n_own, str, lds, n_str, q, statL, statC, strL, strC, part, chunk, blockIdx.x, blockIdx.y);
}

constexpr int W_OWN = 16, W_KL = 16;
constexpr int kMaxWideN = 512;
constexpr int wide_kc(int n) { return n <= 128 ? 8 : (n <= 256 ? 16 : 32); }
constexpr int wide_ts(int kc) { return kc == 32 ? 16 : 32; }
enum WideMode { W_FWD = 0, W_FWD_ROWGRAD = 1, W_BWD_OWNER = 2, W_BWD_STREAM = 3, W_BWD_SYM = 4 };

template <int PK>
__device__ __forceinline__ float term1(float o, float s, const Params& q) {
  if constexpr (PK == PK_DOT) return o * s;
  else if constexpr (PK == 2) { const float d = o - s; return d * d; }
  else if constexpr (PK == 1) return fabsf(o - s);
  else if constexpr (PK == 3) { const float d = o - s; return fabsf(d) * d * d; }
  else { const float a = fabsf(q.sgn * (o - s) + q.eps); return a > 0.f ? fexp2(q.p * flog2(a)) : 0.f; }
}
template <int PK>
__device__ __forceinline__ float dterm1(float o, float s, const Params& q) {
  if constexpr (PK == PK_DOT) return s;
  else if constexpr (PK == 2) return o - s;
  else if constexpr (PK == 1) { const float d = o - s; return d > 0.f ? 1.f : (d < 0.f ? -1.f : 0.f); }
  else if constexpr (PK == 3) { const float d = o - s; return d * fabsf(d); }
  else {
    const float e = q.sgn * (o - s) + q.eps, a = fabsf(e);
    const float v = a > 0.f ? fexp2((q.p - 1.f) * flog2(a)) : 0.f;
    return e < 0.f ? -v : v;
  }
}

template <int KC, int PK, int MODE>
__global__ __launch_bounds__(THREADS) void wide_k(
    const float* __restrict__ own, int64_t ldo, int64_t n_own,
    const float* __restrict__ str, int64_t lds, int64_t n_str, Params q,
    const float* __restrict__ ownL, const float* __restrict__ ownC,
    const float* __restrict__ strL, const float* __restrict__ strC,
    float2* __restrict__ part, float* __restrict__ part_g, int np, int chunk) {
  constexpr bool FWD = MODE == W_FWD || MODE == W_FWD_ROWGRAD, ROWGRAD = MODE == W_FWD_ROWGRAD;
  constexpr bool OWNER_STATS = MODE == W_BWD_OWNER || MODE == W_BWD_SYM, STREAM_STATS = MODE == W_BWD_STREAM || MODE == W_BWD_SYM;
  constexpr bool GRAD = MODE != W_FWD;
  constexpr int TS = wide_ts(KC), LDT = KC * W_KL;
  __shared__ __attribute__((aligned(16))) float tile[TS * LDT];
  __shared__ float tL[TS], tC[TS];
  const int oi = threadIdx.x >> 4, kl = threadIdx.x & (W_KL - 1);
  const int64_t i = (int64_t)blockIdx.x * W_OWN + oi;
  const bool own_ok = i < n_own;
  float o[KC], g[GRAD ? KC : 1];
#pragma unroll
  for (int c = 0; c < KC; ++c) {
    const int k = kl + W_KL * c;
    const bool ok = own_ok && k < q.n;
    const float x = own[ok ? i * ldo + k : 0];
    o[c] = ok ? x : 0.f;
  }
#pragma unroll
  for (int c = 0; c < (GRAD ? KC : 1); ++c) g[c] = 0.f;
  float oL = 0.f, oC = 0.f;
  if (OWNER_STATS && own_ok) { oL = ownL[i]; oC = ownC[i]; }
  float m = -INFINITY, s = 0.f;
  const float xk = q.xs * q.kscale;
  const float csgn = (PK == 0) ? q.sgn : 1.f;
  const bool root = !q.pow;
  const int64_t jb = (int64_t)blockIdx.y * chunk;
  const int64_t je = min(n_str, jb + (int64_t)chunk);
  for (int64_t j0 = jb; j0 < je; j0 += TS) {
    const int cnt = (int)min((int64_t)TS, je - j0);
    __syncthreads();
    for (int idx = threadIdx.x; idx < TS * LDT; idx += THREADS) {
      const int row = idx / LDT, k = idx - row * LDT;
      const bool ok = row < cnt && k < q.n;
      const float x = str[ok ? (j0 + row) * lds + k : 0];
      tile[idx] = ok ? x : 0.f;
    }
    if (STREAM_STATS && (int)threadIdx.x < TS) {
      const bool ok = (int)threadIdx.x < cnt;
      const float l = strL[ok ? j0 + threadIdx.x : 0], c = strC[ok ? j0 + threadIdx.x : 0];
      tL[threadIdx.x] = ok ? l : 0.f; tC[threadIdx.x] = ok ? c : 0.f;
    }
    __syncthreads();
    for (int jj = 0; jj < cnt; ++jj) {
      const float* row = tile + jj * LDT + kl;
      float acc = 0.f;
#pragma unroll
      for (int c = 0; c < KC; ++c)
        if (PK != 0 || kl + W_KL * c < q.n) acc += term1<PK>(o[c], row[W_KL * c], q);
#pragma unroll
      for (int off = W_KL / 2; off > 0; off >>= 1) acc += __shfl_xor(acc, off, 64);
      const float x = (root ? root_of<true>(acc, q) : acc) * xk;
      const float dr = (root ? droot_of<true>(acc, q) : q.p) * csgn;
      float cf;
      if (FWD) {
        const float mn = fmaxf(x, fmaxf(m, -1e30f));
        const float e = fexp2(x - mn), resc = fexp2(m - mn);
        s = fmaf(s, resc, e);
        m = mn;
        cf = e * dr;
        if (ROWGRAD) {
#pragma unroll
          for (int c = 0; c < KC; ++c) g[c] *= resc;
        }
      } else {
        float w = 0.f;
        if (OWNER_STATS) w = oC * fexp2(x - oL);
        if (STREAM_STATS) w = fmaf(tC[jj], fexp2(x - tL[jj]), w);
        cf = w * dr;
      }
      if (GRAD) {
#pragma unroll
        for (int c = 0; c < KC; ++c)
          if (PK != 0 || kl + W_KL * c < q.n) g[c] = fmaf(cf, dterm1<PK>(o[c], row[W_KL * c], q), g[c]);
      }
    }
  }
  if (!own_ok) return;
  const int64_t slot = (int64_t)blockIdx.y * n_own + i;
  if (FWD && kl == 0) part[slot] = make_float2(fmaxf(m, -1e30f), s);
  if (GRAD) {
#pragma unroll
    for (int c = 0; c < KC; ++c) {
      const int k = kl + W_KL * c;
      if (k < np) part_g[slot * np + k] = k < q.n ? g[c] : 0.f;
    }
  }
}

inline int pad_dim(int n) {
  static const int dims[] = {4, 8, 12, 16, 24, 32, 40, 64};
  for (int d : dims) if (n <= d) return d;
  if (n <= kMaxWideN) return (n + 3) / 4 * 4;
  return -1;
}
constexpr int owners_fwd(int np) { return np <= 24 ? 2 : 1; }
constexpr int owners_bwd(int np) { return np <= 16 ? 2 : 1; }

struct Plan {
  int np, R;
  int64_t tiles;
  int nsplit, chunk;
};
inline Plan make_plan(int64_t n_own, int64_t n_str, int n, bool bwd, int resident = 0) {
  Plan P;
  P.np = pad_dim(n);
  if (P.np > 64) {
    const int64_t TSW = wide_ts(wide_kc(n));
    P.R = 0;
    P.tiles = ceil_div(n_own, (int64_t)W_OWN);
    int64_t ns = ceil_div((int64_t)kNumCU * 4, P.tiles);
    const int64_t cap = ceil_div(n_str, TSW);
    if (ns > cap) ns = cap;
    if (ns < 1) ns = 1;
    const int64_t chunk = ceil_div(ceil_div(n_str, ns), TSW) * TSW;
    P.chunk = (int)chunk;
    P.nsplit = (int)ceil_div(n_str, chunk);
    return P;
  }
  P.R = bwd ? owners_bwd(P.np) : owners_fwd(P.np);
  P.tiles = ceil_div(n_own, (int64_t)HALF * P.R);
  const int64_t TS = tile_rows(P.np);
  const int64_t max_split = ceil_div(n_str, TS);
  auto finish = [&](int64_t ns) {
    if (ns < 1) ns = 1;
    if (ns > max_split) ns = max_split;
    int64_t chunk = ceil_div(ceil_div(n_str, ns), TS) * TS;
    if (chunk < TS) chunk = TS;
    P.chunk = (int)chunk;
    P.nsplit = (int)(n_str > 0 ? ceil_div(n_str, chunk) : 1);
  };
  double best = 1e300; int64_t best_ns = 1;
  if (resident < 0) {
    const int64_t lo1 = ceil_div((int64_t)kNumCU * 2, P.tiles), hi1 = ceil_div((int64_t)kNumCU * 6, P.tiles);
    const int64_t h1 = hi1 > max_split ? max_split : (hi1 < 1 ? 1 : hi1);
    const int64_t l1 = lo1 < 1 ? 1 : (lo1 > h1 ? h1 : lo1);
    for (int64_t ns = l1; ns <= h1; ++ns) {
      const int64_t chunk = ceil_div(ceil_div(n_str, ns), TS) * TS;
      const int64_t nsp = ceil_div(n_str, chunk);
      const int64_t rounds = ceil_div(P.tiles * nsp, (int64_t)kNumCU);
      const double cost = (double)rounds * (double)(chunk + 192) * (1.0 + 0.03 * (rounds < 3 ? 3 - rounds : 0)) + 4.0 * (double)nsp;
      if (cost < best - 1e-9) { best = cost; best_ns = nsp; }
    }
    finish(best_ns);
    return P;
  }
  const int64_t RES = resident > 0 ? resident : (P.np <= 16 ? 3 : 2);
  const int64_t slots = (int64_t)kNumCU * RES;
  const int64_t lo = ceil_div(slots, P.tiles), hi = ceil_div(slots * 6, P.tiles);
  const int64_t ns_hi = hi > max_split ? max_split : (hi < 1 ? 1 : hi);
  const int64_t ns_lo = lo < 1 ? 1 : (lo > ns_hi ? ns_hi : lo);
  for (int64_t ns = ns_lo; ns <= ns_hi; ++ns) {
    const int64_t chunk = ceil_div(ceil_div(n_str, ns), TS) * TS;
    const int64_t nsp = ceil_div(n_str, chunk);
    const int64_t rounds = ceil_div(P.tiles * nsp, slots);
    const double cost = ((double)rounds + 0.25) * (double)RES * (double)(chunk + 192) + 4.0 * (double)nsp;
    if (cost < best - 1e-9) { best = cost; best_ns = nsp; }
  }
  finish(best_ns);
  return P;
}


#define CLICA_LP_DECLARE(PKV)                                                                          \
  void launch_fwd_partial_pk##PKV(const Plan& P, const float* own, int64_t ldo, int64_t n_own,        \
                                  const float* str, int64_t lds, int64_t n_str, const Params& q,      \
                                  float2* part, float* part_g, hipStream_t st);                       \
  void launch_bwd_pairs_pk##PKV(const Plan& P, bool owner_stats, const float* own, int64_t ldo,       \
                                int64_t n_own, const float* str, int64_t lds, int64_t n_str,          \
                                const Params& q, const float* statL, const float* statC, float* part, \
                                hipStream_t st);                                                      \
  void launch_bwd_sym_pk##PKV(const Plan& P, const float* own, int64_t ldo, int64_t n_own,            \
                              const float* str, int64_t lds, int64_t n_str, const Params& q,          \
                              const float* ownL, const float* ownC, const float* strL, const float* strC, \
                              float* part, hipStream_t st);
CLICA_LP_DECLARE(0) CLICA_LP_DECLARE(1) CLICA_LP_DECLARE(2) CLICA_LP_DECLARE(3) CLICA_LP_DECLARE(4)

}
}
```

cl_ica_amd/csrc/lp_loss.hip:

```cpp
#include "lp_kernels.h"
#include "lp_finalize.h"
#include "lp_mfma.h"
#include "lp_mfma_dev.h"

namespace clica {
namespace lp {

__global__ __launch_bounds__(64) void means_k(const float* __restrict__ blocksums, int nblocks, float inv_count,
                                              float* __restrict__ means) {
  float v[3] = {0.f, 0.f, 0.f};
  for (int b = threadIdx.x; b < nblocks; b += 64) {
    v[0] += blocksums[b * 3 + 0]; v[1] += blocksums[b * 3 + 1]; v[2] += blocksums[b * 3 + 2];
  }
#pragma unroll
  for (int a = 0; a < 3; ++a) {
#pragma unroll
    for (int off = 32; off > 0; off >>= 1) v[a] += __shfl_down(v[a], off, 64);
  }
  if (threadIdx.x == 0) { means[0] = v[0] * inv_count; means[1] = v[1] * inv_count; means[2] = v[2] * inv_count; }
}

struct FeatOut { lp2::u32x4_t* FP = nullptr; const float* origin = nullptr; float pre2 = 0.f; int64_t pool_tiles = 0; };
struct Gate { float* words = nullptr; float limit = 0.f; int nsplit_alt = 0; };

__global__ __launch_bounds__(THREADS) void fwd_finalize_k(
    const float2* __restrict__ part, int nsplit, int64_t rows,
    const float* __restrict__ z1, int64_t ld1, const float* __restrict__ z2, int64_t ld2,
    Params q, float tau, float alpha, int compat, int frac, int dot, float log_b3,
    float* __restrict__ loss_i, float* __restrict__ pos_i, float* __restrict__ lse_i, Means M, TrainOut T, FeatOut F, Gate G) {
  if (G.words && lp2::guard_falls_back(G.words, G.limit)) {
    nsplit = G.nsplit_alt;
    if (blockIdx.x == 0 && threadIdx.x == 0) G.words[lp2::W_FALLBACKS] += 1.f;
  }
  __shared__ float sm[THREADS / FIN_ROWS][FIN_ROWS], ss[THREADS / FIN_ROWS][FIN_ROWS];
  __shared__ float ush[FIN_ROWS];
  constexpr int FIN_MAXN = 64;
  __shared__ float zrows[2][FIN_ROWS * FIN_MAXN];
  float v_loss, v_pos, v_lse;
  finalize_rows((int)blockIdx.x, part, nsplit, rows, z1, ld1, z2, ld2, q, tau, alpha, compat, frac, dot, log_b3, loss_i, pos_i, lse_i, T,
                FinScratch{&sm[0][0], &ss[0][0], zrows[0], zrows[1], FIN_MAXN, F.FP ? ush : nullptr}, v_loss, v_pos, v_lse);
  if (F.FP) {
    static_assert(THREADS == 2 * 128 && FIN_ROWS == 2 * lp2::ROWS, "a finalize block = two pool tiles of 128 feature vectors each");
    __syncthreads();
    const int id = threadIdx.x;
    const int64_t r0 = (int64_t)blockIdx.x * FIN_ROWS;
    lp2::feat_vectors((int64_t)blockIdx.x * 2 + (id >> 7), (id >> 6) & 1, (id >> 5) & 1, id & 31, rows, q.n, F.origin, F.pre2,
                      [&](int64_t j, int f) { return zrows[0][(j - r0) * q.n + f]; },
                      [&](int64_t j) { return ush[j - r0]; }, F.FP);
    if (blockIdx.x == gridDim.x - 1) {
      const lp2::u32x4_t z4 = {0u, 0u, 0u, 0u};
      for (int64_t v = (int64_t)gridDim.x * 2 * lp2::FEATVEC + id; v < F.pool_tiles * lp2::FEATVEC; v += THREADS) F.FP[v] = z4;
    }
  }
  reduce_means(v_loss, v_pos, v_lse, M, (int)blockIdx.x);
}

__global__ __launch_bounds__(THREADS) void bwd_coef_k(
    int64_t rows, const float* __restrict__ z1, int64_t ld1, const float* __restrict__ z2, int64_t ld2,
    Params q, float tau, float alpha, int compat, int frac, int dot, const float* __restrict__ lse_i,
    const float* __restrict__ g_mean, const float* __restrict__ g_item,
    const float* __restrict__ g_pos, const float* __restrict__ g_neg,
    float* __restrict__ statL, float* __restrict__ statC,
    float* __restrict__ dz1, int64_t ldd1, float* __restrict__ dz2, int64_t ldd2) {
  const int64_t i = (int64_t)blockIdx.x * THREADS + threadIdx.x;
  if (i >= rows) return;
  coef_row(i, rows, z1 + i * ld1, z2 + i * ld2, q, tau, alpha, compat, frac, dot, lse_i[i], g_mean, g_item, g_pos, g_neg, statL, statC,
           dz1, ldd1, dz2, ldd2);
}

struct MeansJob { const float* blocksums; int nblocks; float inv_count; float* means; int block; int32_t* tick; };
__global__ __launch_bounds__(THREADS) void bwd_reduce_k(const float* __restrict__ part, int nsplit, int64_t rows,
                                                       int np, int n, float* __restrict__ out, int64_t ldo,
                                                       int accumulate, MeansJob mj, Gate G) {
  if (G.words && lp2::guard_falls_back(G.words, G.limit)) nsplit = G.nsplit_alt;
  if ((int)blockIdx.x == mj.block) {
    if (threadIdx.x < 64) {
      float v[3] = {0.f, 0.f, 0.f};
      for (int b = threadIdx.x; b < mj.nblocks; b += 64) {
        v[0] += mj.blocksums[b * 3 + 0]; v[1] += mj.blocksums[b * 3 + 1]; v[2] += mj.blocksums[b * 3 + 2];
      }
#pragma unroll
      for (int a = 0; a < 3; ++a)
#pragma unroll
        for (int off = 32; off > 0; off >>= 1) v[a] += __shfl_down(v[a], off, 64);
      if (threadIdx.x == 0) {
        mj.means[0] = v[0] * mj.inv_count; mj.means[1] = v[1] * mj.inv_count; mj.means[2] = v[2] * mj.inv_count;
        if (mj.tick) mj.tick[0] += 1;
      }
    }
    return;
  }
  const int64_t tid = (int64_t)blockIdx.x * THREADS + threadIdx.x;
  const int64_t idx = tid >> 2;
  const int sub = (int)(tid & 3);
  const int q4 = np / 4;
  const bool live = idx < rows * q4;
  const int64_t i = live ? idx / q4 : 0;
  const int k = live ? (int)(idx - i * q4) * 4 : 0;
  const int64_t stride = rows * (int64_t)np;
  const float* src = part + i * np + k;
  float4 t = make_float4(0.f, 0.f, 0.f, 0.f);
  if (live && k < n) {
#pragma unroll 4
    for (int sp = sub; sp < nsplit; sp += 4) {
      const float4 v = *reinterpret_cast<const float4*>(src + (int64_t)sp * stride);
      t.x += v.x; t.y += v.y; t.z += v.z; t.w += v.w;
    }
  }
#pragma unroll
  for (int off = 1; off <= 2; off <<= 1) {
    t.x += __shfl_xor(t.x, off, 64); t.y += __shfl_xor(t.y, off, 64);
    t.z += __shfl_xor(t.z, off, 64); t.w += __shfl_xor(t.w, off, 64);
  }
  if (!live || k >= n || sub != 0) return;
  float* dst = out + i * ldo + k;
  const float tv[4] = {t.x, t.y, t.z, t.w};
#pragma unroll
  for (int u = 0; u < 4; ++u)
    if (k + u < n) dst[u] = accumulate ? (dst[u] + tv[u]) : tv[u];
}

static Params make_params(const clica_lp_loss_desc* d, bool frac) {
  Params q;
  q.p = d->p; q.inv_p = 1.f / d->p; q.kscale = kLog2e / d->tau;
  q.sgn = frac ? -1.f : 1.f; q.eps = frac ? 1e-12f : 0.f; q.xs = -1.f;
  q.pow = d->pow ? 1 : 0; q.n = d->n;
  return q;
}
static constexpr int train_flags() { return 7; }
static int exponent_kind(float p) { return p == 1.f ? 1 : (p == 2.f ? 2 : (p == 3.f ? 3 : 0)); }

static void launch_fwd_partial(const Plan& P, int pk, const float* own, int64_t ldo, int64_t n_own,
                               const float* str, int64_t lds, int64_t n_str, const Params& q,
                               float2* part, float* part_g, hipStream_t st) {
  switch (pk) {
    case 1: launch_fwd_partial_pk1(P, own, ldo, n_own, str, lds, n_str, q, part, part_g, st); break;
    case 2: launch_fwd_partial_pk2(P, own, ldo, n_own, str, lds, n_str, q, part, part_g, st); break;
    case 3: launch_fwd_partial_pk3(P, own, ldo, n_own, str, lds, n_str, q, part, part_g, st); break;
    case 4: launch_fwd_partial_pk4(P, own, ldo, n_own, str, lds, n_str, q, part, part_g, st); break;
    default: launch_fwd_partial_pk0(P, own, ldo, n_own, str, lds, n_str, q, part, part_g, st); break;
  }
}

__global__ __launch_bounds__(THREADS) void rowgrad_combine_k(const float2* __restrict__ part, const float* __restrict__ part_g,
                                                            int nsplit, int64_t rows, int np, int n,
                                                            const float* __restrict__ lse_i, float* __restrict__ rowgrad,
                                                            int64_t ldrg) {
  const int64_t idx = (int64_t)blockIdx.x * THREADS + threadIdx.x;
  const int q4 = np / 4;
  if (idx >= rows * q4) return;
  const int64_t i = idx / q4;
  const int k = (int)(idx - i * q4) * 4;
  if (k >= n) return;
  const float L2 = lse_i[i];
  float4 t = make_float4(0.f, 0.f, 0.f, 0.f);
#pragma unroll 4
  for (int sp = 0; sp < nsplit; ++sp) {
    const float w = fexp2(part[(int64_t)sp * rows + i].x - L2);
    const float4 g = *reinterpret_cast<const float4*>(part_g + ((int64_t)sp * rows + i) * np + k);
    t.x = fmaf(g.x, w, t.x); t.y = fmaf(g.y, w, t.y); t.z = fmaf(g.z, w, t.z); t.w = fmaf(g.w, w, t.w);
  }
  const float tv[4] = {t.x, t.y, t.z, t.w};
#pragma unroll
  for (int u = 0; u < 4; ++u)
    if (k + u < n) rowgrad[i * ldrg + k + u] = tv[u];
}

__global__ __launch_bounds__(THREADS) void rowgrad_apply_k(const float* __restrict__ rowgrad, int64_t ldrg,
                                                          const float* __restrict__ statC, int64_t rows, int n,
                                                          float* __restrict__ out, int64_t ldo, int accumulate) {
  const int64_t idx = (int64_t)blockIdx.x * THREADS + threadIdx.x;
  if (idx >= rows * n) return;
  const int64_t i = idx / n;
  const int k = (int)(idx - i * n);
  const float v = statC[i] * rowgrad[i * ldrg + k];
  float* dst = out + i * ldo + k;
  *dst = accumulate ? (*dst + v) : v;
}
static void launch_bwd_pairs(bool owner_stats, const Plan& P, int pk, const float* own, int64_t ldo, int64_t n_own,
                             const float* str, int64_t lds, int64_t n_str, const Params& q,
                             const float* statL, const float* statC, float* part, hipStream_t st) {
  switch (pk) {
    case 1: launch_bwd_pairs_pk1(P, owner_stats, own, ldo, n_own, str, lds, n_str, q, statL, statC, part, st); break;
    case 2: launch_bwd_pairs_pk2(P, owner_stats, own, ldo, n_own, str, lds, n_str, q, statL, statC, part, st); break;
    case 3: launch_bwd_pairs_pk3(P, owner_stats, own, ldo, n_own, str, lds, n_str, q, statL, statC, part, st); break;
    case 4: launch_bwd_pairs_pk4(P, owner_stats, own, ldo, n_own, str, lds, n_str, q, statL, statC, part, st); break;
    default: launch_bwd_pairs_pk0(P, owner_stats, own, ldo, n_own, str, lds, n_str, q, statL, statC, part, st); break;
  }
}

static void launch_bwd_sym(const Plan& P, int pk, const float* own, int64_t ldo, int64_t n_own, const float* str, int64_t lds,
                           int64_t n_str, const Params& q, const float* ownL, const float* ownC, const float* strL,
                           const float* strC, float* part, hipStream_t st) {
  switch (pk) {
    case 1: launch_bwd_sym_pk1(P, own, ldo, n_own, str, lds, n_str, q, ownL, ownC, strL, strC, part, st); break;
    case 2: launch_bwd_sym_pk2(P, own, ldo, n_own, str, lds, n_str, q, ownL, ownC, strL, strC, part, st); break;
    case 3: launch_bwd_sym_pk3(P, own, ldo, n_own, str, lds, n_str, q, ownL, ownC, strL, strC, part, st); break;
    case 4: launch_bwd_sym_pk4(P, own, ldo, n_own, str, lds, n_str, q, ownL, ownC, strL, strC, part, st); break;
    default: launch_bwd_sym_pk0(P, own, ldo, n_own, str, lds, n_str, q, ownL, ownC, strL, strC, part, st); break;
  }
}

__global__ __launch_bounds__(THREADS) void pool_stats_k(int64_t pool_rows, const float* __restrict__ pool_lse, int64_t local_rows,
                                                       float tau, float alpha, const float* __restrict__ g_mean,
                                                       const float* __restrict__ g_neg, float xs,
                                                       float* __restrict__ strL, float* __restrict__ strC) {
  const int64_t j = (int64_t)blockIdx.x * THREADS + threadIdx.x;
  if (j >= pool_rows) return;
  const float inv = 1.f / (float)local_rows;
  const float C = 2.f * (1.f - alpha) * (g_mean ? g_mean[0] : 1.f) * inv + (g_neg ? g_neg[0] * inv : 0.f);
  strL[j] = pool_lse[j];
  strC[j] = xs * C / tau;
}

struct FwdWs { float2* part; float* part_g; float* blocksums; size_t bytes; };
struct BwdWs { float* statL; float* statC; float* partR; float* partC; size_t bytes; };

constexpr size_t kHeaderBytes = 4096;
constexpr int64_t kArriveMaxTiles = (int64_t)(kHeaderBytes - 64) / 4 - 1;
static int* header_arrive(void* ws) { return reinterpret_cast<int*>((char*)ws + 64); }
static FwdWs carve_fwd(void* ws, const Plan& P, int64_t rows, bool rowgrad) {
  FwdWs w; char* p = (char*)ws; size_t off = 0;
  off += kHeaderBytes;
  w.blocksums = (float*)(p + off); off += align_up((size_t)ceil_div(rows, FIN_ROWS) * 3 * sizeof(float), 256);
  w.part = (float2*)(p + off); off += align_up((size_t)P.nsplit * rows * sizeof(float2), 256);
  w.part_g = nullptr;
  if (rowgrad) { w.part_g = (float*)(p + off); off += align_up((size_t)P.nsplit * rows * P.np * sizeof(float), 256); }
  w.bytes = off; return w;
}
static size_t fwd_carve_max(int64_t rows, int64_t cols, int n) {
  const size_t a = carve_fwd(nullptr, make_plan(rows, cols, n, false), rows, false).bytes;
  const size_t b = carve_fwd(nullptr, make_plan(rows, cols, n, true), rows, true).bytes;
  return a > b ? a : b;
}
static BwdWs carve_bwd(void* ws, const Plan& PR, const Plan& PC, int64_t rows, int64_t cols) {
  BwdWs w; char* p = (char*)ws; size_t off = kHeaderBytes;
  w.statL = (float*)(p + off); off += align_up((size_t)rows * sizeof(float), 256);
  w.statC = (float*)(p + off); off += align_up((size_t)rows * sizeof(float), 256);
  w.partR = (float*)(p + off); off += align_up((size_t)PR.nsplit * rows * PR.np * sizeof(float), 256);
  w.partC = (float*)(p + off); off += align_up((size_t)PC.nsplit * cols * PC.np * sizeof(float), 256);
  w.bytes = off; return w;
}

static int validate(const clica_lp_loss_desc* d, const char* who) {
  CLICA_CHECK_ARG(d != nullptr, "%s: desc is NULL", who);
  CLICA_CHECK_ARG(d->B > 0 && d->B3 > 0, "%s: B=%lld B3=%lld must be positive", who, (long long)d->B, (long long)d->B3);
  CLICA_CHECK_ARG(d->n >= 1, "%s: n=%d must be >= 1", who, d->n);
  CLICA_CHECK_ARG(pad_dim(d->n) > 0, "%s: n=%d > %d (register-resident kernels to 64, wide-row kernels beyond)", who, d->n, kMaxWideN);
  CLICA_CHECK_ARG(d->p > 0.f, "%s: p=%g must be > 0", who, d->p);
  CLICA_CHECK_ARG(d->tau > 0.f, "%s: tau=%g must be > 0", who, d->tau);
  if (d->p < 1.f && !d->no_eps)
    CLICA_CHECK_ARG(d->B == d->B3, "%s: p<1 uses the transposed branch (losses.py:433-442) and needs B3 == B", who);
  return CLICA_OK;
}

}
}

using namespace clica;
using namespace clica::lp;

extern "C" int clica_lp_loss_workspace_bytes(const clica_lp_loss_desc* d, size_t* fwd_bytes, size_t* bwd_bytes) {
  int rc = validate(d, "clica_lp_loss_workspace_bytes");
  if (rc) return rc;
  const bool frac = d->p < 1.f && !d->no_eps;
  const int64_t rows = frac ? d->B3 : d->B, cols = frac ? d->B : d->B3;
  Plan PF = make_plan(rows, cols, d->n, false);
  Plan PR = make_plan(rows, cols, d->n, true);
  Plan PC = make_plan(cols, rows, d->n, true);
  if (fwd_bytes) *fwd_bytes = fwd_carve_max(rows, cols, d->n);
  (void)PF;
  if (bwd_bytes) *bwd_bytes = carve_bwd(nullptr, PR, PC, rows, cols).bytes;
  return CLICA_OK;
}

static int& fused_finalize_switch() { static int on = 1; return on; }
namespace clica { namespace lp { void set_fused_finalize(int on) { fused_finalize_switch() = on ? 1 : 0; } } }
static bool launch_fwd_partial_fin(const Plan& P, int pk, const float* own, int64_t ldo, int64_t n_own, const float* str, int64_t lds,
                                   int64_t n_str, const Params& q, float2* part, const FinArgs& F, hipStream_t st) {
  switch (pk) {
    case 1: return launch_fwd_partial_fin_pk1(P, own, ldo, n_own, str, lds, n_str, q, part, F, st);
    case 2: return launch_fwd_partial_fin_pk2(P, own, ldo, n_own, str, lds, n_str, q, part, F, st);
    case 3: return launch_fwd_partial_fin_pk3(P, own, ldo, n_own, str, lds, n_str, q, part, F, st);
    default: return false;
  }
}
extern "C" int clica_lp_loss_fwd(const clica_lp_loss_desc* d,
                                 const float* z1, int64_t ld1, const float* z2, int64_t ld2,
                                 const float* z3, int64_t ld3,
                                 float* loss_i, float* pos_i, float* lse_i, float* means,
                                 float* rowgrad, int64_t ldrg,
                                 void* workspace, size_t workspace_bytes, clica_stream_t stream) {
  int rc = validate(d, "clica_lp_loss_fwd");
  if (rc) return rc;
  CLICA_CHECK_ARG(z1 && z2 && z3 && loss_i && pos_i && lse_i && means && workspace, "clica_lp_loss_fwd: NULL pointer");
  CLICA_CHECK_ARG(ld1 >= d->n && ld2 >= d->n && ld3 >= d->n, "clica_lp_loss_fwd: leading dimension < n");
  const bool frac = d->p < 1.f && !d->no_eps;
  const float* rows_p = frac ? z3 : z1; const int64_t ldr = frac ? ld3 : ld1; const int64_t rows = frac ? d->B3 : d->B;
  const float* cols_p = frac ? z1 : z3; const int64_t ldc = frac ? ld1 : ld3; const int64_t cols = frac ? d->B : d->B3;
  CLICA_CHECK_ARG(!rowgrad || ldrg >= d->n, "clica_lp_loss_fwd: rowgrad leading dimension < n");
  Plan P = make_plan(rows, cols, d->n, rowgrad != nullptr);
  FwdWs w = carve_fwd(workspace, P, rows, rowgrad != nullptr);
  if (w.bytes > workspace_bytes) { set_error("clica_lp_loss_fwd: workspace %zu < %zu", workspace_bytes, w.bytes); return CLICA_E_WORKSPACE; }
  Params q = make_params(d, frac);
  if (!frac && !rowgrad && z3 == z1 && ld3 == ld1 && d->B3 == d->B && d->pow && exponent_kind(d->p) != 0 && (train_flags() & 1)) {
    q.train = 1;
    if (exponent_kind(d->p) >= 2) q.pre = powf(q.kscale, 1.f / d->p);
  }
  hipStream_t st = as_stream(stream);
  if (fused_finalize_switch() && !frac && !rowgrad && P.tiles <= kArriveMaxTiles &&
      launch_fwd_partial_fin(P, exponent_kind(d->p), rows_p, ldr, rows, cols_p, ldc, cols, q, w.part,
                             FinArgs{z2, ld2, d->tau, d->alpha, d->compat ? 1 : 0, logf((float)cols), loss_i, pos_i, lse_i, Means{w.blocksums},
                                     TrainOut{}, header_arrive(workspace), means, 1.f / (float)rows}, st))
    return launch_status("clica_lp_loss_fwd");
  launch_fwd_partial(P, exponent_kind(d->p), rows_p, ldr, rows, cols_p, ldc, cols, q, w.part, w.part_g, st);
  Means M{w.blocksums};
  const int nfin = (int)ceil_div(rows, FIN_ROWS);
  hipLaunchKernelGGL(fwd_finalize_k, dim3((unsigned)nfin), dim3(THREADS), 0, st,
                     (const float2*)w.part, P.nsplit, rows, z1, ld1, z2, ld2, q, d->tau, d->alpha,
                     d->compat ? 1 : 0, frac ? 1 : 0, 0, logf((float)cols), loss_i, pos_i, lse_i, M, TrainOut{}, FeatOut{}, Gate{});
  hipLaunchKernelGGL(means_k, dim3(1), dim3(64), 0, st, (const float*)w.blocksums, nfin, 1.f / (float)rows, means);
  if (rowgrad)
    hipLaunchKernelGGL(rowgrad_combine_k, dim3((unsigned)ceil_div(rows * (P.np / 4), THREADS)), dim3(THREADS), 0, st,
                       (const float2*)w.part, (const float*)w.part_g, P.nsplit, rows, P.np, d->n, (const float*)lse_i, rowgrad, ldrg);
  return launch_status("clica_lp_loss_fwd");
}

extern "C" int clica_lp_loss_bwd(const clica_lp_loss_desc* d,
                                 const float* z1, int64_t ld1, const float* z2, int64_t ld2,
                                 const float* z3, int64_t ld3, const float* lse_i,
                                 const float* rowgrad, int64_t ldrg,
                                 const float* g_mean, const float* g_item, const float* g_pos, const float* g_neg,
                                 float* dz1, int64_t ldd1, float* dz2, int64_t ldd2,
                                 float* dz3, int64_t ldd3, int32_t accumulate_dz3,
                                 void* workspace, size_t workspace_bytes, clica_stream_t stream) {
  int rc = validate(d, "clica_lp_loss_bwd");
  if (rc) return rc;
  CLICA_CHECK_ARG(z1 && z2 && z3 && lse_i && workspace, "clica_lp_loss_bwd: NULL pointer");
  const bool frac = d->p < 1.f && !d->no_eps;
  const int64_t rows = frac ? d->B3 : d->B, cols = frac ? d->B : d->B3;
  const float* rows_p = frac ? z3 : z1; const int64_t ldr = frac ? ld3 : ld1;
  const float* cols_p = frac ? z1 : z3; const int64_t ldc = frac ? ld1 : ld3;
  float* d_rows = frac ? dz3 : dz1; const int64_t ld_dr = frac ? ldd3 : ldd1;
  float* d_cols = frac ? dz1 : dz3; const int64_t ld_dc = frac ? ldd1 : ldd3;
  Plan PR = make_plan(rows, cols, d->n, true);
  Plan PC = make_plan(cols, rows, d->n, true);
  BwdWs w = carve_bwd(workspace, PR, PC, rows, cols);
  if (w.bytes > workspace_bytes) { set_error("clica_lp_loss_bwd: workspace %zu < %zu", workspace_bytes, w.bytes); return CLICA_E_WORKSPACE; }
  Params q = make_params(d, frac);
  const int pk = exponent_kind(d->p);
  hipStream_t st = as_stream(stream);
  hipLaunchKernelGGL(bwd_coef_k, dim3((unsigned)ceil_div(rows, THREADS)), dim3(THREADS), 0, st,
                     rows, z1, ld1, z2, ld2, q, d->tau, d->alpha, d->compat ? 1 : 0, frac ? 1 : 0, 0, lse_i,
                     g_mean, g_item, g_pos, g_neg, w.statL, w.statC, dz1, ldd1, dz2, ldd2);
  if (d_rows && rowgrad) {
    const int acc = frac ? (accumulate_dz3 ? 1 : 0) : 1;
    hipLaunchKernelGGL(rowgrad_apply_k, dim3((unsigned)ceil_div(rows * d->n, THREADS)), dim3(THREADS), 0, st,
                       rowgrad, ldrg, (const float*)w.statC, rows, d->n, d_rows, ld_dr, acc);
  } else if (d_rows) {
    launch_bwd_pairs(true, PR, pk, rows_p, ldr, rows, cols_p, ldc, cols, q, w.statL, w.statC, w.partR, st);
    const int acc = frac ? (accumulate_dz3 ? 1 : 0) : 1;
    hipLaunchKernelGGL(bwd_reduce_k, dim3((unsigned)ceil_div(rows * PR.np, THREADS)), dim3(THREADS), 0, st,
                       (const float*)w.partR, PR.nsplit, rows, PR.np, d->n, d_rows, ld_dr, acc, MeansJob{nullptr, 0, 0.f, nullptr, -1, nullptr}, Gate{});
  }
  if (d_cols) {
    Params qc = q; qc.sgn = -q.sgn;
    launch_bwd_pairs(false, PC, pk, cols_p, ldc, cols, rows_p, ldr, rows, qc, w.statL, w.statC, w.partC, st);
    const int acc = frac ? 1 : (accumulate_dz3 ? 1 : 0);
    hipLaunchKernelGGL(bwd_reduce_k, dim3((unsigned)ceil_div(cols * PC.np, THREADS)), dim3(THREADS), 0, st,
                       (const float*)w.partC, PC.nsplit, cols, PC.np, d->n, d_cols, ld_dc, acc, MeansJob{nullptr, 0, 0.f, nullptr, -1, nullptr}, Gate{});
  }
  return launch_status("clica_lp_loss_bwd");
}

extern "C" int clica_lp_loss_bwd_sym(const clica_lp_loss_desc* d,
                                     const float* z1, int64_t ld1, const float* z2, int64_t ld2,
                                     const float* pool, int64_t ldp, const float* lse_i, const float* pool_lse,
                                     const float* g_mean, const float* g_pos, const float* g_neg,
                                     float* dz1, int64_t ldd1, float* dz2, int64_t ldd2,
                                     void* workspace, size_t workspace_bytes, clica_stream_t stream) {
  int rc = validate(d, "clica_lp_loss_bwd_sym");
  if (rc) return rc;
  CLICA_CHECK_ARG(z1 && z2 && pool && lse_i && pool_lse && dz1 && workspace, "clica_lp_loss_bwd_sym: NULL pointer");
  CLICA_CHECK_ARG(d->p >= 1.f || d->no_eps, "clica_lp_loss_bwd_sym: the p<1 branch is not symmetric (eps inside the abs, losses.py:436)");
  CLICA_CHECK_ARG(d->B3 >= d->B, "clica_lp_loss_bwd_sym: the pool (B3=%lld rows) must contain the %lld local rows", (long long)d->B3, (long long)d->B);
  const int64_t rows = d->B, cols = d->B3;
  Plan PR = make_plan(rows, cols, d->n, true);
  Plan PC = make_plan(cols, rows, d->n, true);
  BwdWs w = carve_bwd(workspace, PR, PC, rows, cols);
  if (w.bytes > workspace_bytes) { set_error("clica_lp_loss_bwd_sym: workspace %zu < %zu", workspace_bytes, w.bytes); return CLICA_E_WORKSPACE; }
  float* strL = w.partC;
  float* strC = w.partC + cols;
  Params q = make_params(d, false);
  hipStream_t st = as_stream(stream);
  hipLaunchKernelGGL(bwd_coef_k, dim3((unsigned)ceil_div(rows, THREADS)), dim3(THREADS), 0, st,
                     rows, z1, ld1, z2, ld2, q, d->tau, d->alpha, d->compat ? 1 : 0, 0, 0, lse_i,
                     g_mean, (const float*)nullptr, g_pos, g_neg, w.statL, w.statC, dz1, ldd1, dz2, ldd2);
  if (pool_lse == lse_i && cols == rows) {
    strL = w.statL; strC = w.statC;
  } else {
    hipLaunchKernelGGL(pool_stats_k, dim3((unsigned)ceil_div(cols, THREADS)), dim3(THREADS), 0, st,
                       cols, pool_lse, rows, d->tau, d->alpha, g_mean, g_neg, q.xs, strL, strC);
  }
  Params qs = q;
  if ((train_flags() & 2) && exponent_kind(d->p) != 0 && d->pow) {
    qs.train = 2;
    if (exponent_kind(d->p) >= 2) qs.pre = powf(qs.kscale, 1.f / d->p);
    qs.gfold = d->p / powf(qs.pre, d->p - 1.f);
  }
  launch_bwd_sym(PR, exponent_kind(d->p), z1, ld1, rows, pool, ldp, cols, qs, w.statL, w.statC, strL, strC, w.partR, st);
  hipLaunchKernelGGL(bwd_reduce_k, dim3((unsigned)ceil_div(rows * PR.np, THREADS)), dim3(THREADS), 0, st,
                     (const float*)w.partR, PR.nsplit, rows, PR.np, d->n, dz1, ldd1, 1, MeansJob{nullptr, 0, 0.f, nullptr, -1, nullptr}, Gate{});
  return launch_status("clica_lp_loss_bwd_sym");
}

struct TrainWs { float* blocksums; int* arrive; float* statL; float* statC; float* strL; float* strC; char* scratch; size_t scratch_bytes; size_t bytes;
                 bool mfma; lp2::Plan P2; lp2::Ws w2; };
static bool train_mfma_shape(const clica_lp_loss_desc* d) { return (train_flags() & 7) == 7 && lp2::applies(d->n, d->p, d->pow); }
static bool train_mfma(const clica_lp_loss_desc* d) { return train_mfma_shape(d) && lp2::applies_to_pool(d->B, d->B3); }
static TrainWs carve_train(void* ws, const Plan& PF, const Plan& PR, int64_t rows, int64_t cols, bool mfma) {
  TrainWs w; char* p = (char*)ws; size_t off = kHeaderBytes;
  w.blocksums = (float*)(p + off); off += align_up((size_t)ceil_div(rows, FIN_ROWS) * 3 * sizeof(float), 256);
  w.arrive = (int*)(p + off); off += align_up((size_t)ceil_div(rows, FIN_ROWS) * sizeof(int), 256);
  w.statL = (float*)(p + off); off += align_up((size_t)rows * sizeof(float), 256);
  w.statC = (float*)(p + off); off += align_up((size_t)rows * sizeof(float), 256);
  w.strL = (float*)(p + off); off += align_up((size_t)cols * sizeof(float), 256);
  w.strC = (float*)(p + off); off += align_up((size_t)cols * sizeof(float), 256);
  w.mfma = mfma;
  int nsf = PF.nsplit, nsr = PR.nsplit;
  if (mfma) {
    w.P2 = lp2::make_plan(rows, cols);
    w.w2 = lp2::carve(p + off, w.P2);
    off += w.w2.bytes;
    nsf = w.P2.nsplit > nsf ? w.P2.nsplit : nsf;
    nsr = w.P2.nsplit > nsr ? w.P2.nsplit : nsr;
  }
  w.scratch = p + off;
  const size_t f = align_up((size_t)nsf * rows * sizeof(float2), 256);
  const size_t b = align_up((size_t)nsr * rows * PR.np * sizeof(float), 256);
  w.scratch_bytes = f > b ? f : b;
  w.bytes = off + w.scratch_bytes; return w;
}

extern "C" int clica_lp_loss_train_workspace_bytes(const clica_lp_loss_desc* d, size_t* bytes) {
  int rc = validate(d, "clica_lp_loss_train_workspace_bytes");
  if (rc) return rc;
  CLICA_CHECK_ARG(bytes != nullptr, "clica_lp_loss_train_workspace_bytes: bytes is NULL");
  *bytes = carve_train(nullptr, make_plan(d->B, d->B3, d->n, false), make_plan(d->B, d->B3, d->n, true), d->B, d->B3, train_mfma_shape(d)).bytes;
  return CLICA_OK;
}

extern "C" int clica_lp_loss_train_path(const clica_lp_loss_desc* d, int32_t* path) {
  int rc = validate(d, "clica_lp_loss_train_path");
  if (rc) return rc;
  CLICA_CHECK_ARG(path != nullptr, "clica_lp_loss_train_path: path is NULL");
  *path = train_mfma(d) ? 1 : 0;
  return CLICA_OK;
}

extern "C" int clica_lp_loss_set_matrix_cores(int32_t on) {
  lp2::set_enabled(on);
  return CLICA_OK;
}

extern "C" int clica_lp_loss_train_spread(const clica_lp_loss_desc* d, const void* workspace, size_t workspace_bytes, float* spread,
                                          clica_stream_t stream) {
  int rc = validate(d, "clica_lp_loss_train_spread");
  if (rc) return rc;
  CLICA_CHECK_ARG(workspace && spread, "clica_lp_loss_train_spread: NULL pointer");
  *spread = 0.f;
  if (!train_mfma(d)) return CLICA_OK;
  const int64_t rows = d->B, cols = d->B3;
  TrainWs w = carve_train(const_cast<void*>(workspace), make_plan(rows, cols, d->n, false), make_plan(rows, cols, d->n, true), rows, cols, true);
  if (w.bytes > workspace_bytes) { set_error("clica_lp_loss_train_spread: workspace %zu < %zu", workspace_bytes, w.bytes); return CLICA_E_WORKSPACE; }
  hipStream_t st = as_stream(stream);
  if (hipMemcpyAsync(spread, w.w2.spread, sizeof(float), hipMemcpyDeviceToHost, st) != hipSuccess || hipStreamSynchronize(st) != hipSuccess)
    return launch_status("clica_lp_loss_train_spread");
  return CLICA_OK;
}

extern "C" int clica_lp_loss_set_spread_limit(float limit) {
  lp2::set_spread_limit(limit);
  return CLICA_OK;
}

extern "C" int clica_lp_loss_train_guard(const clica_lp_loss_desc* d, const void* workspace, size_t workspace_bytes, float* out4,
                                         clica_stream_t stream) {
  int rc = validate(d, "clica_lp_loss_train_guard");
  if (rc) return rc;
  CLICA_CHECK_ARG(workspace && out4, "clica_lp_loss_train_guard: NULL pointer");
  out4[0] = out4[1] = out4[3] = 0.f; out4[2] = lp2::spread_limit();
  if (!train_mfma(d)) return CLICA_OK;
  const int64_t rows = d->B, cols = d->B3;
  TrainWs w = carve_train(const_cast<void*>(workspace), make_plan(rows, cols, d->n, false), make_plan(rows, cols, d->n, true), rows, cols, true);
  if (w.bytes > workspace_bytes) { set_error("clica_lp_loss_train_guard: workspace %zu < %zu", workspace_bytes, w.bytes); return CLICA_E_WORKSPACE; }
  hipStream_t st = as_stream(stream);
  float words[16];
  if (hipMemcpyAsync(words, w.w2.spread, sizeof(words), hipMemcpyDeviceToHost, st) != hipSuccess || hipStreamSynchronize(st) != hipSuccess)
    return launch_status("clica_lp_loss_train_guard");
  out4[0] = words[lp2::W_RUN_M]; out4[1] = words[lp2::W_M64]; out4[3] = words[lp2::W_FALLBACKS];
  return CLICA_OK;
}

namespace clica { namespace lp {
constexpr unsigned kTrainStateVersion = 1u;
constexpr int kTrainStateWords = 64;
constexpr size_t kTrainStateBytes = (4 + kTrainStateWords) * sizeof(unsigned);
__global__ __launch_bounds__(64) void train_state_export_k(const unsigned* __restrict__ words, unsigned* __restrict__ blob) {
  const int t = threadIdx.x;
  if (t < 4) blob[t] = t == 0 ? kTrainStateVersion : (t == 1 ? (unsigned)kTrainStateWords : 0u);
  if (t < kTrainStateWords) blob[4 + t] = words[t];
}
__global__ __launch_bounds__(64) void train_state_import_k(unsigned* __restrict__ words, const unsigned* __restrict__ blob) {
  const int t = threadIdx.x;
  if (t < kTrainStateWords) words[t] = blob[4 + t];
}
} }
extern "C" int clica_lp_loss_train_state_bytes(size_t* bytes) {
  CLICA_CHECK_ARG(bytes != nullptr, "clica_lp_loss_train_state_bytes: bytes is NULL");
  *bytes = kTrainStateBytes;
  return CLICA_OK;
}
extern "C" int clica_lp_loss_train_state_export(const clica_lp_loss_desc* d, const void* workspace, size_t workspace_bytes, void* blob,
                                                size_t blob_bytes, clica_stream_t stream) {
  int rc = validate(d, "clica_lp_loss_train_state_export");
  if (rc) return rc;
  CLICA_CHECK_ARG(workspace && blob, "clica_lp_loss_train_state_export: NULL pointer");
  CLICA_CHECK_ARG(blob_bytes >= kTrainStateBytes, "clica_lp_loss_train_state_export: blob of %zu bytes < %zu", blob_bytes, kTrainStateBytes);
  hipStream_t st = as_stream(stream);
  if (!train_mfma(d)) {
    if (hipMemsetAsync(blob, 0, kTrainStateBytes, st) != hipSuccess) return launch_status("clica_lp_loss_train_state_export");
    return CLICA_OK;
  }
  const int64_t rows = d->B, cols = d->B3;
  TrainWs w = carve_train(const_cast<void*>(workspace), make_plan(rows, cols, d->n, false), make_plan(rows, cols, d->n, true), rows, cols, true);
  if (w.bytes > workspace_bytes) { set_error("clica_lp_loss_train_state_export: workspace %zu < %zu", workspace_bytes, w.bytes); return CLICA_E_WORKSPACE; }
  hipLaunchKernelGGL(train_state_export_k, dim3(1), dim3(64), 0, st, reinterpret_cast<const unsigned*>(w.w2.spread), reinterpret_cast<unsigned*>(blob));
  return launch_status("clica_lp_loss_train_state_export");
}
extern "C" int clica_lp_loss_train_state_import(const clica_lp_loss_desc* d, void* workspace, size_t workspace_bytes, const void* blob,
                                                size_t blob_bytes, clica_stream_t stream) {
  int rc = validate(d, "clica_lp_loss_train_state_import");
  if (rc) return rc;
  CLICA_CHECK_ARG(workspace && blob, "clica_lp_loss_train_state_import: NULL pointer");
  CLICA_CHECK_ARG(blob_bytes >= kTrainStateBytes, "clica_lp_loss_train_state_import: blob of %zu bytes < %zu", blob_bytes, kTrainStateBytes);
  if (!train_mfma_shape(d)) return CLICA_OK;
  const int64_t rows = d->B, cols = d->B3;
  TrainWs w = carve_train(workspace, make_plan(rows, cols, d->n, false), make_plan(rows, cols, d->n, true), rows, cols, true);
  if (w.bytes > workspace_bytes) { set_error("clica_lp_loss_train_state_import: workspace %zu < %zu", workspace_bytes, w.bytes); return CLICA_E_WORKSPACE; }
  hipStream_t st = as_stream(stream);
  unsigned head[4];
  if (hipMemcpyAsync(head, blob, sizeof(head), hipMemcpyDeviceToHost, st) != hipSuccess || hipStreamSynchronize(st) != hipSuccess)
    return launch_status("clica_lp_loss_train_state_import");
  if (head[0] == 0u) return CLICA_OK;
  CLICA_CHECK_ARG(head[0] == kTrainStateVersion && head[1] == (unsigned)kTrainStateWords,
                  "clica_lp_loss_train_state_import: blob layout version %u with %u words (this library reads version %u, %d words)",
                  head[0], head[1], kTrainStateVersion, kTrainStateWords);
  hipLaunchKernelGGL(train_state_import_k, dim3(1), dim3(64), 0, st, reinterpret_cast<unsigned*>(w.w2.spread), reinterpret_cast<const unsigned*>(blob));
  return launch_status("clica_lp_loss_train_state_import");
}

extern "C" int clica_lp_loss_fwd_train(const clica_lp_loss_desc* d,
                                       const float* z1, int64_t ld1, const float* z2, int64_t ld2, const float* pool, int64_t ldp,
                                       float* loss_i, float* pos_i, float* lse_i,
                                       float* dz1, int64_t ldd1, float* dz2, int64_t ldd2,
                                       void* workspace, size_t workspace_bytes, clica_stream_t stream) {
  int rc = validate(d, "clica_lp_loss_fwd_train");
  if (rc) return rc;
  CLICA_CHECK_ARG(z1 && z2 && pool && loss_i && pos_i && lse_i && dz1 && dz2 && workspace, "clica_lp_loss_fwd_train: NULL pointer");
  CLICA_CHECK_ARG(d->p >= 1.f, "clica_lp_loss_fwd_train: the p<1 branch is not symmetric (eps inside the abs, losses.py:436)");
  CLICA_CHECK_ARG(ld1 >= d->n && ld2 >= d->n && ldp >= d->n && ldd1 >= d->n && ldd2 >= d->n, "clica_lp_loss_fwd_train: leading dimension < n");
  const int64_t rows = d->B, cols = d->B3;
  Plan PF = make_plan(rows, cols, d->n, false), PR = make_plan(rows, cols, d->n, true);
  TrainWs w = carve_train(workspace, PF, PR, rows, cols, train_mfma(d));
  if (w.bytes > workspace_bytes) { set_error("clica_lp_loss_fwd_train: workspace %zu < %zu", workspace_bytes, w.bytes); return CLICA_E_WORKSPACE; }
  Params q = make_params(d, false);
  q.train = train_flags() & 1;
  if (q.train && exponent_kind(d->p) >= 2 && d->pow) q.pre = powf(q.kscale, 1.f / d->p);
  hipStream_t st = as_stream(stream);
  float2* part = reinterpret_cast<float2*>(w.scratch);
// ... 441 lines not shown
```

cl_ica_amd/csrc/lp_loss_pk.hip:

```cpp
#include "lp_kernels.h"
#include "lp_finalize.h"
#include <stdlib.h>
#ifndef CLICA_PK
#error "compile with -DCLICA_PK=0|1|2|3|4"
#endif
#define CAT_(a, b) a##b
#define CAT(a, b) CAT_(a, b)

namespace clica {
namespace lp {

#define LP_FOR_NP(NPV, BODY)                        \
  switch (NPV) {                                    \
    case 4: { constexpr int NP = 4; constexpr int NQ = NP / 2; BODY } break;   \
    case 8: { constexpr int NP = 8; constexpr int NQ = NP / 2; BODY } break;   \
    case 12: if (q.n <= 10) { constexpr int NP = 12; constexpr int NQ = 5; BODY }    \
             else { constexpr int NP = 12; constexpr int NQ = 6; BODY } break; \
    case 16: { constexpr int NP = 16; constexpr int NQ = NP / 2; BODY } break; \
    case 24: { constexpr int NP = 24; constexpr int NQ = NP / 2; BODY } break; \
    case 32: { constexpr int NP = 32; constexpr int NQ = NP / 2; BODY } break; \
    case 40: { constexpr int NP = 40; constexpr int NQ = NP / 2; BODY } break; \
    case 64: { constexpr int NP = 64; constexpr int NQ = NP / 2; BODY } break; \
    default: break;                                 \
  }

template <int PK, int MODE>
static void launch_wide(const Plan& P, const float* own, int64_t ldo, int64_t n_own, const float* str, int64_t lds, int64_t n_str,
                        const Params& q, const float* ownL, const float* ownC, const float* strL, const float* strC,
                        float2* part, float* part_g, hipStream_t st) {
  dim3 grid((unsigned)P.tiles, (unsigned)P.nsplit), block(THREADS);
  switch (wide_kc(q.n)) {
    case 8: hipLaunchKernelGGL((wide_k<8, PK, MODE>), grid, block, 0, st, own, ldo, n_own, str, lds, n_str, q, ownL, ownC, strL, strC, part, part_g, P.np, P.chunk); break;
    case 16: hipLaunchKernelGGL((wide_k<16, PK, MODE>), grid, block, 0, st, own, ldo, n_own, str, lds, n_str, q, ownL, ownC, strL, strC, part, part_g, P.np, P.chunk); break;
    default: hipLaunchKernelGGL((wide_k<32, PK, MODE>), grid, block, 0, st, own, ldo, n_own, str, lds, n_str, q, ownL, ownC, strL, strC, part, part_g, P.np, P.chunk); break;
  }
}

void CAT(launch_fwd_partial_pk, CLICA_PK)(const Plan& P, const float* own, int64_t ldo, int64_t n_own,
                                          const float* str, int64_t lds, int64_t n_str, const Params& q,
                                          float2* part, float* part_g, hipStream_t st) {
  constexpr int PK = CLICA_PK;
  if (P.np > 64) {
    if (part_g) launch_wide<PK, W_FWD_ROWGRAD>(P, own, ldo, n_own, str, lds, n_str, q, nullptr, nullptr, nullptr, nullptr, part, part_g, st);
    else launch_wide<PK, W_FWD>(P, own, ldo, n_own, str, lds, n_str, q, nullptr, nullptr, nullptr, nullptr, part, part_g, st);
    return;
  }
  dim3 grid((unsigned)P.tiles, (unsigned)P.nsplit), block(THREADS);
  LP_FOR_NP(P.np, {
    if (part_g && q.pow)
      hipLaunchKernelGGL((fwd_partial_k<NP, PK, owners_bwd(NP), false, true, NQ>), grid, block, 0, st, own, ldo, n_own, str, lds,
                         n_str, q, part, part_g, P.chunk);
    else if (part_g)
      hipLaunchKernelGGL((fwd_partial_k<NP, PK, owners_bwd(NP), true, true, NQ>), grid, block, 0, st, own, ldo, n_own, str, lds,
                         n_str, q, part, part_g, P.chunk);
    else if (q.pow && (q.train & 1) && PK >= 1 && PK <= 3)
      hipLaunchKernelGGL((fwd_partial_k<NP, PK, owners_fwd(NP), false, false, NQ, (PK >= 1 && PK <= 3)>), grid, block, 0, st, own, ldo, n_own, str, lds,
                         n_str, q, part, part_g, P.chunk);
    else if (q.pow)
      hipLaunchKernelGGL((fwd_partial_k<NP, PK, owners_fwd(NP), false, false, NQ>), grid, block, 0, st, own, ldo, n_own, str, lds,
                         n_str, q, part, part_g, P.chunk);
    else
      hipLaunchKernelGGL((fwd_partial_k<NP, PK, owners_fwd(NP), true, false, NQ>), grid, block, 0, st, own, ldo, n_own, str, lds,
                         n_str, q, part, part_g, P.chunk);
  })
}

bool CAT(launch_fwd_partial_fin_pk, CLICA_PK)(const Plan& P, const float* own, int64_t ldo, int64_t n_own,
                                              const float* str, int64_t lds, int64_t n_str, const Params& q,
                                              float2* part, const FinArgs& F, hipStream_t st) {
  constexpr int PK = CLICA_PK;
  if constexpr (PK >= 1 && PK <= 3) {
    if (P.np > 16) return false;
    dim3 grid((unsigned)P.tiles, (unsigned)P.nsplit), block(THREADS);
    bool done = false;
    LP_FOR_NP(P.np, {
      if constexpr (NP <= 16 && HALF * owners_fwd(NP) == FIN_ROWS) {
        if (q.pow && (q.train & 1))
          hipLaunchKernelGGL((fwd_partial_fin_k<NP, PK, owners_fwd(NP), false, NQ, true>), grid, block, 0, st, own, ldo, n_own, str, lds,
                             n_str, q, part, P.chunk, F);
        else if (q.pow)
          hipLaunchKernelGGL((fwd_partial_fin_k<NP, PK, owners_fwd(NP), false, NQ, false>), grid, block, 0, st, own, ldo, n_own, str, lds,
                             n_str, q, part, P.chunk, F);
        else
          hipLaunchKernelGGL((fwd_partial_fin_k<NP, PK, owners_fwd(NP), true, NQ, false>), grid, block, 0, st, own, ldo, n_own, str, lds,
                             n_str, q, part, P.chunk, F);
        done = true;
      }
    })
    return done;
  }
  return false;
}

void CAT(launch_bwd_pairs_pk, CLICA_PK)(const Plan& P, bool owner_stats, const float* own, int64_t ldo,
                                        int64_t n_own, const float* str, int64_t lds, int64_t n_str,
                                        const Params& q, const float* statL, const float* statC, float* part,
                                        hipStream_t st) {
  constexpr int PK = CLICA_PK;
  if (P.np > 64) {
    if (owner_stats) launch_wide<PK, W_BWD_OWNER>(P, own, ldo, n_own, str, lds, n_str, q, statL, statC, nullptr, nullptr, nullptr, part, st);
    else launch_wide<PK, W_BWD_STREAM>(P, own, ldo, n_own, str, lds, n_str, q, nullptr, nullptr, statL, statC, nullptr, part, st);
    return;
  }
  dim3 grid((unsigned)P.tiles, (unsigned)P.nsplit), block(THREADS);
  LP_FOR_NP(P.np, {
    if (owner_stats && q.pow)
      hipLaunchKernelGGL((bwd_pairs_k<NP, PK, owners_bwd(NP), 1, false, NQ>), grid, block, 0, st, own, ldo, n_own, str,
                         lds, n_str, q, statL, statC, statL, statC, part, P.chunk);
    else if (owner_stats)
      hipLaunchKernelGGL((bwd_pairs_k<NP, PK, owners_bwd(NP), 1, true, NQ>), grid, block, 0, st, own, ldo, n_own, str,
                         lds, n_str, q, statL, statC, statL, statC, part, P.chunk);
    else if (q.pow)
      hipLaunchKernelGGL((bwd_pairs_k<NP, PK, owners_bwd(NP), 2, false, NQ>), grid, block, 0, st, own, ldo, n_own, str,
                         lds, n_str, q, statL, statC, statL, statC, part, P.chunk);
    else
      hipLaunchKernelGGL((bwd_pairs_k<NP, PK, owners_bwd(NP), 2, true, NQ>), grid, block, 0, st, own, ldo, n_own, str,
                         lds, n_str, q, statL, statC, statL, statC, part, P.chunk);
  })
}

void CAT(launch_bwd_sym_pk, CLICA_PK)(const Plan& P, const float* own, int64_t ldo, int64_t n_own,
                                      const float* str, int64_t lds, int64_t n_str, const Params& q,
                                      const float* ownL, const float* ownC, const float* strL, const float* strC,
                                      float* part, hipStream_t st) {
  constexpr int PK = CLICA_PK;
  if (P.np > 64) {
    launch_wide<PK, W_BWD_SYM>(P, own, ldo, n_own, str, lds, n_str, q, ownL, ownC, strL, strC, nullptr, part, st);
    return;
  }
  dim3 grid((unsigned)P.tiles, (unsigned)P.nsplit), block(THREADS);
  LP_FOR_NP(P.np, {
    if (q.pow && (q.train & 2) && PK >= 1 && PK <= 3)
      hipLaunchKernelGGL((bwd_pairs_k<NP, PK, owners_bwd(NP), 3, false, NQ, (PK >= 1 && PK <= 3)>), grid, block, 0, st, own, ldo, n_own, str,
                         lds, n_str, q, ownL, ownC, strL, strC, part, P.chunk);
    else if (q.pow)
      hipLaunchKernelGGL((bwd_pairs_k<NP, PK, owners_bwd(NP), 3, false, NQ>), grid, block, 0, st, own, ldo, n_own, str,
                         lds, n_str, q, ownL, ownC, strL, strC, part, P.chunk);
    else
      hipLaunchKernelGGL((bwd_pairs_k<NP, PK, owners_bwd(NP), 3, true, NQ>), grid, block, 0, st, own, ldo, n_own, str,
                         lds, n_str, q, ownL, ownC, strL, strC, part, P.chunk);
  })
}

}
}
```

cl_ica_amd/csrc/nn_search.hip:

```cpp
#include "lp_kernels.h"
#include <limits.h>

namespace clica {
namespace nn {
using namespace clica::lp;

__device__ __forceinline__ bool before(float d, int j, float d2, int j2) { return d < d2 || (d == d2 && j < j2); }

template <int K>
__device__ __forceinline__ void insert(float (&bd)[K], int (&bi)[K], float d, int j) {
  if (!before(d, j, bd[K - 1], bi[K - 1])) return;
  bd[K - 1] = d; bi[K - 1] = j;
#pragma unroll
  for (int c = K - 1; c > 0; --c) {
    if (before(bd[c], bi[c], bd[c - 1], bi[c - 1])) {
      const float td = bd[c]; bd[c] = bd[c - 1]; bd[c - 1] = td;
      const int ti = bi[c]; bi[c] = bi[c - 1]; bi[c - 1] = ti;
    }
  }
}

struct Cand { float d; int i; };

template <int NP, int R, int K, int NQ = NP / 2>
__global__ __launch_bounds__(THREADS) void nn_partial_k(const float* __restrict__ qry, int64_t ldq, int64_t n_q,
                                                       const float* __restrict__ tab, int64_t ldt, int64_t n_tab,
                                                       Params q, Cand* __restrict__ part, int chunk) {
  constexpr int TS = tile_rows(NP), RPP = TS / PARTS;
  __shared__ __attribute__((aligned(16))) float tiles[2][TS * NP];
  __shared__ Cand wred[WAVES][HALF * R][K];
  const int lane = threadIdx.x & 63, wave = threadIdx.x >> 6, li = lane & (HALF - 1), hf = lane >> 5;
  const int pq = wave * 2 + hf;
  const int64_t own0 = (int64_t)blockIdx.x * (HALF * R);
  f32x2 o[R][NP / 2];
  load_owners<NP, R>(o, qry, ldq, own0, n_q, q.n);
  float bd[R][K]; int bi[R][K];
#pragma unroll
  for (int r = 0; r < R; ++r)
#pragma unroll
    for (int c = 0; c < K; ++c) { bd[r][c] = INFINITY; bi[r][c] = INT_MAX; }

  const int64_t jb = (int64_t)blockIdx.y * chunk;
  const int64_t je = min(n_tab, jb + (int64_t)chunk);
  Stager<NP> st;
  if (jb < je) {
    st.load(tab, ldt, jb, (int)min((int64_t)TS, je - jb), q.n);
    st.store(tiles[0]);
  }
  __syncthreads();
  int cur = 0;
  for (int64_t j0 = jb; j0 < je; j0 += TS, cur ^= 1) {
    const int cnt = (int)min((int64_t)TS, je - j0);
    const bool more = j0 + TS < je;
    if (more) st.load(tab, ldt, j0 + TS, (int)min((int64_t)TS, je - j0 - TS), q.n);
    const float* tile = tiles[cur] + pq * RPP * NP;
    const int cq = min(RPP, max(0, cnt - pq * RPP));
    const int row0 = (int)j0 + pq * RPP;
    for (int jj = 0; jj < cq; jj += JB) {
#pragma unroll
      for (int r = 0; r < R; ++r) {
        float acc[JB];
        dist_group<NP, 2, NQ>(o[r], tile, jj, q, acc);
        const float worst = bd[r][K - 1];
        const float best4 = fminf(fminf(acc[0], acc[1]), fminf(acc[2], acc[3]));
        if (best4 < worst || jj + JB > cq) {
#pragma unroll
          for (int c = 0; c < JB; ++c)
            if (jj + c < cq) insert<K>(bd[r], bi[r], acc[c], row0 + jj + c);
        }
      }
    }
    if (more) st.store(tiles[cur ^ 1]);
    __syncthreads();
  }
#pragma unroll
  for (int r = 0; r < R; ++r) {
    float od[K]; int oi[K];
#pragma unroll
    for (int c = 0; c < K; ++c) { od[c] = __shfl_xor(bd[r][c], HALF, 64); oi[c] = __shfl_xor(bi[r][c], HALF, 64); }
#pragma unroll
    for (int c = 0; c < K; ++c) insert<K>(bd[r], bi[r], od[c], oi[c]);
    if (hf == 0) {
#pragma unroll
      for (int c = 0; c < K; ++c) wred[wave][r * HALF + li][c] = Cand{bd[r][c], bi[r][c]};
    }
  }
  __syncthreads();
  if (threadIdx.x < HALF * R) {
    const int t = threadIdx.x;
    const int64_t i = own0 + t;
    float md[K]; int mi[K];
#pragma unroll
    for (int c = 0; c < K; ++c) { md[c] = wred[0][t][c].d; mi[c] = wred[0][t][c].i; }
#pragma unroll
    for (int w = 1; w < WAVES; ++w)
#pragma unroll
      for (int c = 0; c < K; ++c) insert<K>(md, mi, wred[w][t][c].d, wred[w][t][c].i);
    if (i < n_q) {
#pragma unroll
      for (int c = 0; c < K; ++c) part[((int64_t)blockIdx.y * n_q + i) * K + c] = Cand{md[c], mi[c]};
    }
  }
}

template <int K>
__global__ __launch_bounds__(THREADS) void nn_merge_k(const Cand* __restrict__ part, int nsplit, int64_t n_q, int k,
                                                     int64_t* __restrict__ idx, float* __restrict__ dist) {
  const int64_t i = (int64_t)blockIdx.x * THREADS + threadIdx.x;
  if (i >= n_q) return;
  float md[K]; int mi[K];
#pragma unroll
  for (int c = 0; c < K; ++c) { md[c] = INFINITY; mi[c] = INT_MAX; }
  for (int sp = 0; sp < nsplit; ++sp)
#pragma unroll
    for (int c = 0; c < K; ++c) {
      const Cand v = part[((int64_t)sp * n_q + i) * K + c];
      insert<K>(md, mi, v.d, v.i);
    }
#pragma unroll
  for (int c = 0; c < K; ++c)
    if (c < k) {
      idx[i * k + c] = mi[c] == INT_MAX ? -1 : (int64_t)mi[c];
      if (dist) dist[i * k + c] = md[c];
    }
}

template <int K>
static void launch(const Plan& P, const float* qry, int64_t ldq, int64_t n_q, const float* tab, int64_t ldt, int64_t n_tab,
                   const Params& q, Cand* part, int k, int64_t* idx, float* dist, hipStream_t st) {
  dim3 grid((unsigned)P.tiles, (unsigned)P.nsplit), block(THREADS);
#define NN_CASE(NPV, NQV)                                                                                              \
  hipLaunchKernelGGL((nn_partial_k<NPV, owners_fwd(NPV), K, NQV>), grid, block, 0, st, qry, ldq, n_q, tab, ldt, n_tab, q, part, P.chunk)
  switch (P.np) {
    case 4: NN_CASE(4, 2); break;
    case 8: NN_CASE(8, 4); break;
    case 12: if (q.n <= 10) NN_CASE(12, 5); else NN_CASE(12, 6); break;
    case 16: NN_CASE(16, 8); break;
    case 24: NN_CASE(24, 12); break;
    case 32: NN_CASE(32, 16); break;
    case 40: NN_CASE(40, 20); break;
    default: NN_CASE(64, 32); break;
  }
#undef NN_CASE
  hipLaunchKernelGGL((nn_merge_k<K>), dim3((unsigned)ceil_div(n_q, THREADS)), dim3(THREADS), 0, st, (const Cand*)part, P.nsplit,
                     n_q, k, idx, dist);
}

constexpr int kMaxK = 4;
constexpr int kResident = -1;
static int kcap(int k) { return k <= 1 ? 1 : (k <= 2 ? 2 : 4); }
}
}

using namespace clica;

extern "C" int clica_nn_search_workspace_bytes(int64_t n_query, int64_t n_table, int32_t n, int32_t k, size_t* bytes) {
  CLICA_CHECK_ARG(bytes && n_query > 0 && n_table > 0 && n >= 1 && n <= 64 && k >= 1 && k <= nn::kMaxK,
                  "clica_nn_search_workspace_bytes: need n_query, n_table > 0, 1 <= n <= 64, 1 <= k <= %d", nn::kMaxK);
  const lp::Plan P = lp::make_plan(n_query, n_table, n, false, nn::kResident);
  *bytes = align_up((size_t)P.nsplit * n_query * nn::kcap(k) * sizeof(nn::Cand), 256);
  return CLICA_OK;
}

extern "C" int clica_nn_search(const float* table, int64_t ldt, int64_t n_table, const float* query, int64_t ldq, int64_t n_query,
                               int32_t n, int32_t k, int64_t* idx, float* dist, void* workspace, size_t workspace_bytes,
                               clica_stream_t stream) {
  CLICA_CHECK_ARG(table && query && idx && workspace && n_query > 0 && n_table > 0, "clica_nn_search: bad argument");
  CLICA_CHECK_ARG(n >= 1 && n <= 64 && ldt >= n && ldq >= n, "clica_nn_search: n=%d must be in 1..64 and <= the leading dimensions", n);
  CLICA_CHECK_ARG(k >= 1 && k <= nn::kMaxK, "clica_nn_search: k=%d must be in 1..%d", k, nn::kMaxK);
  CLICA_CHECK_ARG(n_table < (int64_t)INT_MAX, "clica_nn_search: table rows are indexed with 32 bits on chip");
  size_t need = 0;
  clica_nn_search_workspace_bytes(n_query, n_table, n, k, &need);
  if (need > workspace_bytes) { set_error("clica_nn_search: workspace %zu < %zu", workspace_bytes, need); return CLICA_E_WORKSPACE; }
  const lp::Plan P = lp::make_plan(n_query, n_table, n, false, nn::kResident);
  lp::Params q;
  q.p = 2.f; q.inv_p = 0.5f; q.kscale = 1.f; q.sgn = 1.f; q.eps = 0.f; q.xs = -1.f; q.pow = 1; q.n = n;
  hipStream_t st = as_stream(stream);
  nn::Cand* part = reinterpret_cast<nn::Cand*>(workspace);
  switch (nn::kcap(k)) {
    case 1: nn::launch<1>(P, query, ldq, n_query, table, ldt, n_table, q, part, k, idx, dist, st); break;
    case 2: nn::launch<2>(P, query, ldq, n_query, table, ldt, n_table, q, part, k, idx, dist, st); break;
    default: nn::launch<4>(P, query, ldq, n_query, table, ldt, n_table, q, part, k, idx, dist, st); break;
  }
  return launch_status("clica_nn_search");
}
```

Measured before the change: 2811.

## Precompute stager offsets, register-resident finalize rows, split cap knob, trace hooks

The tile stager now precomputes per-thread 32-bit byte offsets once per chunk and advances a base pointer, so the per-tile address math and the 64-bit multiplies disappear from the streaming loop. The pre-scale and bounds masking move from load to store. The fused finalize gets a register path (templated on NP) that reads staged rows from LDS once into registers and specialises the p-norm and gradient loops. The change also adds an lp_max_splits tuning knob and compile-time-gated cycle-counter tracing. It risks extra register pressure from the per-thread offset and flag arrays, and a slower fallback path for wide strides.

```diff
diff --git a/cl_ica_amd/csrc/linear.hip b/cl_ica_amd/csrc/linear.hip
--- a/cl_ica_amd/csrc/linear.hip
+++ b/cl_ica_amd/csrc/linear.hip
@@ -1371,7 +1371,7 @@
   return CLICA_OK;
 }
 
-namespace clica { namespace lp { void set_dot_mfma(int on); void set_fused_finalize(int on); } }
+namespace clica { namespace lp { void set_dot_mfma(int on); void set_fused_finalize(int on); void set_max_splits(int k); } }
 namespace clica { namespace wsplit { void set_epi_specialised(int on); } }
 extern "C" int clica_set_tuning(const char* key, int32_t value) {
   CLICA_CHECK_ARG(key != nullptr, "clica_set_tuning: key is NULL");
@@ -1383,7 +1383,8 @@
   else if (!strcmp(key, "dot_mfma")) clica::lp::set_dot_mfma(value);
   else if (!strcmp(key, "gemm16_epilogue")) clica::wsplit::set_epi_specialised(value);
   else if (!strcmp(key, "lp_fused_finalize")) clica::lp::set_fused_finalize(value);
-  else if (!strcmp(key, "reset")) { t = gemm::Tuning{-1, -1, -1, true}; clica::lp::set_dot_mfma(1); clica::wsplit::set_epi_specialised(1); clica::lp::set_fused_finalize(1); }
+  else if (!strcmp(key, "lp_max_splits")) clica::lp::set_max_splits(value);
+  else if (!strcmp(key, "reset")) { t = gemm::Tuning{-1, -1, -1, true}; clica::lp::set_dot_mfma(1); clica::wsplit::set_epi_specialised(1); clica::lp::set_fused_finalize(1); clica::lp::set_max_splits(0); }
   else { set_error("clica_set_tuning: unknown key '%s'", key); return CLICA_E_INVALID; }
   return CLICA_OK;
 }
diff --git a/cl_ica_amd/csrc/lp_finalize.h b/cl_ica_amd/csrc/lp_finalize.h
--- a/cl_ica_amd/csrc/lp_finalize.h
+++ b/cl_ica_amd/csrc/lp_finalize.h
@@ -19,6 +19,38 @@
   return s;
 }
 
+
+__device__ __forceinline__ float unfused(float t) { asm("" : "+v"(t)); return t; }
+typedef const __attribute__((address_space(3))) float* lds_cfloat_ptr;
+template <int W>
+__device__ __forceinline__ void read_staged_row(float (&r)[W], const float* row, int n) {
+  lds_cfloat_ptr p = (lds_cfloat_ptr)row;
+#pragma unroll
+  for (int k = 0; k < W; ++k) r[k] = p[k < n ? k : 0];
+}
+template <int W>
+__device__ __forceinline__ float pos_sum_regs(const float (&a)[W], const float (&b)[W], int n, const Params& q) {
+  float s = 0.f;
+  if (q.p == 2.f) {
+#pragma unroll
+    for (int k = 0; k < W; ++k) { const float d = a[k] - b[k]; const float t = unfused(d * d); s = k < n ? s + t : s; }
+  } else if (q.p == 1.f) {
+#pragma unroll
+    for (int k = 0; k < W; ++k) { const float d = a[k] - b[k]; const float t = fabsf(d); s = k < n ? s + t : s; }
+  } else if (q.p == 3.f) {
+#pragma unroll
+    for (int k = 0; k < W; ++k) { const float d = a[k] - b[k]; const float t = unfused(fabsf(d) * d * d); s = k < n ? s + t : s; }
+  } else {
+#pragma unroll
+    for (int k = 0; k < W; ++k) {
+      const float d = a[k] - b[k];
+      const float t = fabsf(d) > 0.f ? fexp2(q.p * flog2(fabsf(d))) : 0.f;
+      s = k < n ? s + t : s;
+    }
+  }
+  return s;
+}
+
 struct Means {
   float* blocksums;
 };
@@ -45,6 +77,14 @@
 
 constexpr int FIN_ROWS = 64;
 struct TrainOut { float* statL; float* statC; float* dz1; int64_t ldd1; float* dz2; int64_t ldd2; };
+
+__device__ __forceinline__ float cpos_of(const float sp_, const float A, const float C, const Params& q, float tau, int compat, const float L2) {
+  const float pos = q.pow ? sp_ : root_of<true>(sp_, q);
+  float cpos = A / tau;
+  if (compat) cpos -= (C / tau) * fexp2(-pos * q.kscale - L2);
+  cpos *= q.pow ? q.p : droot_of<true>(sp_, q);
+  return cpos;
+}
 
 __device__ __forceinline__ void coef_row(
     const int64_t i, const int64_t rows, const float* a , const float* b ,
@@ -75,10 +115,7 @@
     return;
   }
   const float sp_ = pos_sum(a, b, q.n, q, frac != 0);
-  const float pos = q.pow ? sp_ : root_of<true>(sp_, q);
-  float cpos = A / tau;
-  if (compat) cpos -= (C / tau) * fexp2(-pos * q.kscale - L2);
-  cpos *= q.pow ? q.p : droot_of<true>(sp_, q);
+  const float cpos = cpos_of(sp_, A, C, q, tau, compat, L2);
   for (int k = 0; k < q.n; ++k) {
     const float d = a[k] - b[k];
     float dt;
@@ -99,9 +136,53 @@
   }
 }
 
+template <int W>
+__device__ __forceinline__ void coef_row_regs(
+    const int64_t i, const int64_t rows, const float (&a)[W], const float (&b)[W], const float sp_,
+    const Params& q, float tau, float alpha, int compat, const float L2,
+    float* __restrict__ statL, float* __restrict__ statC,
+    float* __restrict__ dz1, int64_t ldd1, float* __restrict__ dz2, int64_t ldd2, float* statC_value) {
+  const float inv_rows = 1.f / (float)rows;
+  const float gi = 1.f * inv_rows + 0.f;
+  const float A = 2.f * alpha * gi + 0.f;
+  const float C = 2.f * (1.f - alpha) * gi + 0.f;
+  statL[i] = L2;
+  const float sc = q.xs * C / tau;
+  statC[i] = sc;
+  *statC_value = sc;
+  if (!dz1 && !dz2) return;
+  const float cpos = cpos_of(sp_, A, C, q, tau, compat, L2);
+  const int n = q.n;
+  auto put = [&](int k, float dt) {
+    const float g = cpos * dt;
+    if (k < n) {
+      if (dz1) dz1[i * ldd1 + k] = g;
+      if (dz2) dz2[i * ldd2 + k] = -g;
+    }
+  };
+  if (q.p == 2.f) {
+#pragma unroll
+    for (int k = 0; k < W; ++k) { const float d = a[k] - b[k]; put(k, d); }
+  } else if (q.p == 1.f) {
+#pragma unroll
+    for (int k = 0; k < W; ++k) { const float d = a[k] - b[k]; put(k, (d > 0.f ? 1.f : 0.f) - (d < 0.f ? 1.f : 0.f)); }
+  } else if (q.p == 3.f) {
+#pragma unroll
+    for (int k = 0; k < W; ++k) { const float d = a[k] - b[k]; put(k, d * fabsf(d)); }
+  } else {
+#pragma unroll
+    for (int k = 0; k < W; ++k) {
+      const float d = a[k] - b[k];
+      const float ad = fabsf(d);
+      const float v = ad > 0.f ? fexp2((q.p - 1.f) * flog2(ad)) : 0.f;
+      put(k, d < 0.f ? -v : v);
+    }
+  }
+}
+
 
 struct FinScratch { float* sm; float* ss; float* zr0; float* zr1; int zmaxn; float* ush; };
-template <bool COHERENT = false>
+template <bool COHERENT = false, int W = 0>
 __device__ __forceinline__ void finalize_rows(
     const int blk, const float2* __restrict__ part, const int nsplit, const int64_t rows,
     const float* __restrict__ z1, int64_t ld1, const float* __restrict__ z2, int64_t ld2,
@@ -156,6 +237,11 @@
     float pos, xp;
     const float* ra = staged ? &S.zr0[lane_row * q.n] : z1 + i * ld1;
     const float* rb = staged ? &S.zr1[lane_row * q.n] : z2 + i * ld2;
+    const bool regs = W > 0 && staged && !dot && !frac;
+    float av[W > 0 ? W : 1], bv[W > 0 ? W : 1], sp_regs = 0.f;
+    if constexpr (W > 0) {
+      if (regs) { read_staged_row<W>(av, &S.zr0[lane_row * q.n], q.n); read_staged_row<W>(bv, &S.zr1[lane_row * q.n], q.n); }
+    }
     if (dot) {
       pos = 0.f;
       if (q.posdot) pos = q.posdot[i];
@@ -163,7 +249,10 @@
       xp = pos * q.kscale;
       pos = -pos;
     } else {
-      const float sp_ = pos_sum(ra, rb, q.n, q, frac != 0);
+      float sp_;
+      if constexpr (W > 0) sp_ = regs ? pos_sum_regs<W>(av, bv, q.n, q) : pos_sum(ra, rb, q.n, q, frac != 0);
+      else sp_ = pos_sum(ra, rb, q.n, q, frac != 0);
+      sp_regs = sp_;
       pos = q.pow ? sp_ : root_of<true>(sp_, q);
       xp = -pos * q.kscale;
     }
@@ -179,9 +268,15 @@
     const float li = 2.f * (alpha * lp + (1.f - alpha) * lse);
     loss_i[i] = li; pos_i[i] = lp; lse_i[i] = L2;
     float sc_i = 0.f;
-    if (T.statL)
-      coef_row(i, rows, ra, rb, q, tau, alpha, compat, frac, dot, L2, nullptr, nullptr, nullptr, nullptr, T.statL, T.statC,
-               T.dz1, T.ldd1, T.dz2, T.ldd2, &sc_i);
+    if (T.statL) {
+      bool done = false;
+      if constexpr (W > 0) {
+        if (regs) { coef_row_regs<W>(i, rows, av, bv, sp_regs, q, tau, alpha, compat, L2, T.statL, T.statC, T.dz1, T.ldd1, T.dz2, T.ldd2, &sc_i); done = true; }
+      }
+      if (!done)
+        coef_row(i, rows, ra, rb, q, tau, alpha, compat, frac, dot, L2, nullptr, nullptr, nullptr, nullptr, T.statL, T.statC,
+                 T.dz1, T.ldd1, T.dz2, T.ldd2, &sc_i);
+    }
     v_loss = li; v_pos = lp; v_lse = lse;
     if (S.ush) S.ush[lane_row] = sc_i * fexp2(-L2);
   } else if (S.ush && grp == 0) {
@@ -212,14 +307,17 @@
     if (s_last) __hip_atomic_store(&F.arrive[blockIdx.x], 0, __ATOMIC_RELAXED, __HIP_MEMORY_SCOPE_AGENT);
   }
   __syncthreads();
-  if (!s_last) return;
+  LPT_STAMP(4);
+  if (!s_last) { LPT_FLUSH(0); return; }
   float v_loss, v_pos, v_lse;
   constexpr int ZMAXN = 2 * tile_rows(NP) * NP / (2 * FIN_ROWS);
   static_assert(ZMAXN >= NP, "tile buffers too small for the z rows");
-  finalize_rows<true>((int)blockIdx.x, part, (int)gridDim.y, n_own, own, ldo, F.z2, F.ld2, q, F.tau, F.alpha, F.compat, 0, 0, F.log_b3,
+  finalize_rows<true, NP>((int)blockIdx.x, part, (int)gridDim.y, n_own, own, ldo, F.z2, F.ld2, q, F.tau, F.alpha, F.compat, 0, 0, F.log_b3,
                 F.loss_i, F.pos_i, F.lse_i, F.T, FinScratch{&sm[0][0], &ss[0][0], scratch, scratch + FIN_ROWS * ZMAXN, ZMAXN, nullptr},
                 v_loss, v_pos, v_lse);
   reduce_means(v_loss, v_pos, v_lse, F.M, (int)blockIdx.x, F.means != nullptr);
+  LPT_STAMP(5);
+  LPT_FLUSH(0);
   if (!F.means) return;
   __builtin_amdgcn_s_waitcnt(0x0F70);
   __syncthreads();
diff --git a/cl_ica_amd/csrc/lp_kernels.h b/cl_ica_amd/csrc/lp_kernels.h
--- a/cl_ica_amd/csrc/lp_kernels.h
+++ b/cl_ica_amd/csrc/lp_kernels.h
@@ -122,19 +122,57 @@
   static constexpr int ITERS = TS * NP / THREADS;
   static_assert((TS * NP) % THREADS == 0, "tile must divide over the workgroup");
   float v[ITERS];
-  __device__ __forceinline__ void load(const float* __restrict__ str, int64_t lds, int64_t j0, int cnt, int n, float pre = 1.f) {
+  unsigned off[ITERS];
+  bool kok[ITERS];
+  const float* base;
+  int64_t ld;
+  int cnt;
+  int nn;
+  bool wide;
+  __device__ __forceinline__ void init(const float* __restrict__ str, int64_t lds, int64_t j0, int n) {
+    base = str + j0 * lds; ld = lds; cnt = 0; nn = n;
+    wide = lds > (int64_t)(0x7fffffff / (4 * TS));
 #pragma unroll
     for (int it = 0; it < ITERS; ++it) {
       const int idx = threadIdx.x + it * THREADS;
       const int row = idx / NP, k = idx - row * NP;
-      const bool ok = row < cnt && k < n;
-      const float x = str[ok ? (j0 + row) * lds + k : 0];
-      v[it] = ok ? x * pre : 0.f;
-    }
-  }
-  __device__ __forceinline__ void store(float* tile) const {
-#pragma unroll
-    for (int it = 0; it < ITERS; ++it) tile[threadIdx.x + it * THREADS] = v[it];
+      kok[it] = k < n;
+      off[it] = kok[it] ? ((unsigned)row * (unsigned)lds + (unsigned)k) * 4u : 0u;
+    }
+  }
+  __device__ __forceinline__ void load(int c) {
+    const char* b = reinterpret_cast<const char*>(base);
+    cnt = c;
+    if (!wide) {
+      if (c == TS) {
+#pragma unroll
+        for (int it = 0; it < ITERS; ++it) v[it] = *reinterpret_cast<const float*>(b + off[it]);
+      } else {
+        const unsigned end = (unsigned)c * (unsigned)ld * 4u;
+#pragma unroll
+        for (int it = 0; it < ITERS; ++it) v[it] = *reinterpret_cast<const float*>(b + (off[it] < end ? off[it] : 0u));
+      }
+    }
+    base += (int64_t)TS * ld;
+  }
+  __device__ __forceinline__ void store(float* tile, float pre = 1.f) const {
+    if (wide) {
+      const float* b = base - (int64_t)TS * ld;
+#pragma unroll 1
+      for (int idx = threadIdx.x; idx < TS * NP; idx += THREADS) {
+        const int row = idx / NP, k = idx - row * NP;
+        const bool ok = k < nn && row < cnt;
+        const float x = b[ok ? (int64_t)row * ld + k : 0];
+        tile[idx] = ok ? x * pre : 0.f;
+      }
+    } else if (cnt == TS) {
+#pragma unroll
+      for (int it = 0; it < ITERS; ++it) tile[threadIdx.x + it * THREADS] = kok[it] ? v[it] * pre : 0.f;
+    } else {
+      const unsigned end = (unsigned)cnt * (unsigned)ld * 4u;
+#pragma unroll
+      for (int it = 0; it < ITERS; ++it) tile[threadIdx.x + it * THREADS] = (kok[it] && off[it] < end) ? v[it] * pre : 0.f;
+    }
   }
 };
 
@@ -216,6 +254,24 @@
     g = __builtin_elementwise_fma(c2, t, g);
   }
 }
+
+#ifdef CLICA_LP_TRACE
+static __device__ unsigned long long* g_lp_trace = nullptr;
+constexpr int LPT_MAXWG = 1024, LPT_MAXT = 8, LPT_HEAD = 8, LPT_NS = LPT_HEAD + 4 * LPT_MAXT;
+__device__ __forceinline__ unsigned long long* lpt_buf() { __shared__ unsigned long long b[LPT_NS]; return b; }
+#define LPT_INIT() do { if (threadIdx.x == 0) { for (int i_ = 0; i_ < LPT_NS; ++i_) lpt_buf()[i_] = 0; lpt_buf()[0] = __builtin_readcyclecounter(); } } while (0)
+#define LPT_STAMP(slot) do { if (threadIdx.x == 0) lpt_buf()[slot] = __builtin_readcyclecounter(); } while (0)
+#define LPT_TILE(t, ph) do { if (threadIdx.x == 0 && (t) < LPT_MAXT) lpt_buf()[LPT_HEAD + 4 * (t) + (ph)] = __builtin_readcyclecounter(); } while (0)
+#define LPT_FLUSH(kind) do { if (threadIdx.x == 0 && g_lp_trace) { \
+    const unsigned wg_ = blockIdx.y * gridDim.x + blockIdx.x; \
+    lpt_buf()[6] = __builtin_readcyclecounter(); \
+    if (wg_ < (unsigned)LPT_MAXWG) for (int i_ = 0; i_ < LPT_NS; ++i_) g_lp_trace[((size_t)(kind) * LPT_MAXWG + wg_) * LPT_NS + i_] = lpt_buf()[i_]; } } while (0)
+#else
+#define LPT_INIT() do { } while (0)
+#define LPT_STAMP(slot) do { } while (0)
+#define LPT_TILE(t, ph) do { } while (0)
+#define LPT_FLUSH(kind) do { } while (0)
+#endif
 
 constexpr int fwd_min_waves(int np, bool rowgrad) { return rowgrad ? (np <= 16 ? 3 : 2) : (np <= 16 ? 4 : (np <= 24 ? 3 : 2)); }
 constexpr int bwd_min_waves(int np) { return np <= 16 ? 3 : 2; }
@@ -237,7 +293,9 @@
   const int64_t own0 = (int64_t)bx * (HALF * R);
   f32x2 o[R][NP / 2];
   f32x2 G[ROWGRAD ? R : 1][NP / 2];
+  LPT_INIT();
   load_owners<NP, R>(o, own, ldo, own0, n_own, q.n, q.pre);
+  LPT_STAMP(1);
   float m[R], s[R];
   const float csgn = (PK == 0) ? q.sgn : 1.f;
 #pragma unroll
@@ -253,15 +311,18 @@
   const int64_t je = min(n_str, jb + (int64_t)chunk);
   Stager<NP> st;
   if (jb < je) {
-    st.load(str, lds, jb, (int)min((int64_t)TS, je - jb), q.n, q.pre);
-    st.store(tiles[0]);
+    st.init(str, lds, jb, q.n);
+    st.load((int)min((int64_t)TS, je - jb));
+    st.store(tiles[0], q.pre);
   }
   __syncthreads();
+  LPT_STAMP(2);
   int cur = 0;
   for (int64_t j0 = jb; j0 < je; j0 += TS, cur ^= 1) {
     const int cnt = (int)min((int64_t)TS, je - j0);
     const bool more = j0 + TS < je;
-    if (more) st.load(str, lds, j0 + TS, (int)min((int64_t)TS, je - j0 - TS), q.n, q.pre);
+    if (more) st.load((int)min((int64_t)TS, je - j0 - TS));
+    LPT_TILE((int)((j0 - jb) / TS), 0);
     const float* tile = tiles[cur] + pq * RPP * NP;
     const int cq = min(RPP, max(0, cnt - pq * RPP));
     auto sweep = [&](auto ragged_tag) {
@@ -313,9 +374,12 @@
       }
     }
     };
+    LPT_TILE((int)((j0 - jb) / TS), 1);
     if (cq == RPP) sweep(std::false_type{}); else sweep(std::true_type{});
-    if (more) st.store(tiles[cur ^ 1]);
+    LPT_TILE((int)((j0 - jb) / TS), 2);
+    if (more) st.store(tiles[cur ^ 1], q.pre);
     __syncthreads();
+    LPT_TILE((int)((j0 - jb) / TS), 3);
   }
   float* gred = &tiles[0][0];
 #pragma unroll
@@ -378,6 +442,8 @@
       }
     }
   }
+  LPT_STAMP(3);
+  if (!scratch_out) LPT_FLUSH(0);
 }
 
 template <int NP, int PK, int R, bool ROOT, bool ROWGRAD, int NQ = NP / 2, bool ZMAX = false>
@@ -404,7 +470,9 @@
   const int pq = wave * 2 + hf;
   const int64_t own0 = (int64_t)bx * (HALF * R);
   f32x2 o[R][NP / 2], g[R][NP / 2];
+  LPT_INIT();
   load_owners<NP, R>(o, own, ldo, own0, n_own, q.n, q.pre);
+  LPT_STAMP(1);
   float oL[R], oC[R];
 #pragma unroll
   for (int r = 0; r < R; ++r) {
@@ -424,28 +492,33 @@
   auto load_stats = [&](int64_t j0, int cnt) {
     if (STREAM_STATS && (int)threadIdx.x < TS) {
       const bool ok = (int)threadIdx.x < cnt;
-      const float l = strL[ok ? j0 + threadIdx.x : 0], c = strC[ok ? j0 + threadIdx.x : 0];
-      rl = ok ? l : 0.f;
-      rc = ok ? c : 0.f;
+      rl = strL[ok ? j0 + threadIdx.x : 0]; rc = strC[ok ? j0 + threadIdx.x : 0];
     }
   };
   auto store_stats = [&](int b) {
-    if (STREAM_STATS && (int)threadIdx.x < TS) { tLs[b][threadIdx.x] = rl; tCs[b][threadIdx.x] = FOLD ? rc * fexp2(-rl) * q.gfold : rc; }
+    if (STREAM_STATS && (int)threadIdx.x < TS) {
+      const bool ok = (int)threadIdx.x < st.cnt;
+      const float l = ok ? rl : 0.f, c = ok ? rc : 0.f;
+      tLs[b][threadIdx.x] = l; tCs[b][threadIdx.x] = FOLD ? c * fexp2(-l) * q.gfold : c;
+    }
   };
   if (jb < je) {
     const int c0 = (int)min((int64_t)TS, je - jb);
-    st.load(str, lds, jb, c0, q.n, q.pre); load_stats(jb, c0);
-    st.store(tiles[0]); store_stats(0);
+    st.init(str, lds, jb, q.n);
+    st.load(c0); load_stats(jb, c0);
+    st.store(tiles[0], q.pre); store_stats(0);
   }
   __syncthreads();
+  LPT_STAMP(2);
   int cur = 0;
   for (int64_t j0 = jb; j0 < je; j0 += TS, cur ^= 1) {
     const int cnt = (int)min((int64_t)TS, je - j0);
     const bool more = j0 + TS < je;
     if (more) {
       const int c1 = (int)min((int64_t)TS, je - j0 - TS);
-      st.load(str, lds, j0 + TS, c1, q.n, q.pre); load_stats(j0 + TS, c1);
-    }
+      st.load(c1); load_stats(j0 + TS, c1);
+    }
+    LPT_TILE((int)((j0 - jb) / TS), 0);
     const float* tile = tiles[cur] + pq * RPP * NP;
     const float* tL = tLs[cur] + pq * RPP;
     const float* tC = tCs[cur] + pq * RPP;
@@ -455,6 +528,7 @@
 #endif
     constexpr bool KEEPD = PK >= 1 && PK <= 3 && (NP <= 16 || (CLICA_LP_KEEPD_WIDE && NP <= 40));
     constexpr int JW = KEEPD ? 1 : JBW;
+    LPT_TILE((int)((j0 - jb) / TS), 1);
     for (int jj = 0; jj < cq; jj += JW) {
 #pragma unroll
       for (int r = 0; r < R; ++r) {
@@ -502,8 +576,10 @@
         }
       }
     }
-    if (more) { st.store(tiles[cur ^ 1]); store_stats(cur ^ 1); }
+    LPT_TILE((int)((j0 - jb) / TS), 2);
+    if (more) { st.store(tiles[cur ^ 1], q.pre); store_stats(cur ^ 1); }
     __syncthreads();
+    LPT_TILE((int)((j0 - jb) / TS), 3);
   }
   float* gred = &tiles[0][0];
 #pragma unroll
@@ -535,6 +611,8 @@
     }
     *reinterpret_cast<float4*>(part + ((int64_t)by * n_own + i) * NP + 4 * k4) = a4;
   }
+  LPT_STAMP(3);
+  LPT_FLUSH(1);
 }
 
 template <int NP, int PK, int R, int STATS, bool ROOT, int NQ = NP / 2, bool FOLD = false>
@@ -683,9 +761,11 @@
   int64_t tiles;
   int nsplit, chunk;
 };
+int max_splits_cap();
 inline Plan make_plan(int64_t n_own, int64_t n_str, int n, bool bwd, int resident = 0) {
   Plan P;
   P.np = pad_dim(n);
+  const int64_t cap_ns = max_splits_cap();
   if (P.np > 64) {
     const int64_t TSW = wide_ts(wide_kc(n));
     P.R = 0;
@@ -693,6 +773,7 @@
     int64_t ns = ceil_div((int64_t)kNumCU * 4, P.tiles);
     const int64_t cap = ceil_div(n_str, TSW);
     if (ns > cap) ns = cap;
+    if (cap_ns > 0 && ns > cap_ns) ns = cap_ns;
     if (ns < 1) ns = 1;
     const int64_t chunk = ceil_div(ceil_div(n_str, ns), TSW) * TSW;
     P.chunk = (int)chunk;
@@ -704,6 +785,7 @@
   const int64_t TS = tile_rows(P.np);
   const int64_t max_split = ceil_div(n_str, TS);
   auto finish = [&](int64_t ns) {
+    if (cap_ns > 0 && ns > cap_ns) ns = cap_ns;
     if (ns < 1) ns = 1;
     if (ns > max_split) ns = max_split;
     int64_t chunk = ceil_div(ceil_div(n_str, ns), TS) * TS;
diff --git a/cl_ica_amd/csrc/lp_loss.hip b/cl_ica_amd/csrc/lp_loss.hip
--- a/cl_ica_amd/csrc/lp_loss.hip
+++ b/cl_ica_amd/csrc/lp_loss.hip
@@ -276,6 +276,11 @@
 
 static int& fused_finalize_switch() { static int on = 1; return on; }
 namespace clica { namespace lp { void set_fused_finalize(int on) { fused_finalize_switch() = on ? 1 : 0; } } }
+static int& max_splits_switch() { static int cap = 0; return cap; }
+namespace clica { namespace lp {
+void set_max_splits(int k) { max_splits_switch() = k > 0 ? k : 0; }
+int max_splits_cap() { return max_splits_switch(); }
+} }
 static bool launch_fwd_partial_fin(const Plan& P, int pk, const float* own, int64_t ldo, int64_t n_own, const float* str, int64_t lds,
                                    int64_t n_str, const Params& q, float2* part, const FinArgs& F, hipStream_t st) {
   switch (pk) {
diff --git a/cl_ica_amd/csrc/lp_loss_pk.hip b/cl_ica_amd/csrc/lp_loss_pk.hip
--- a/cl_ica_amd/csrc/lp_loss_pk.hip
+++ b/cl_ica_amd/csrc/lp_loss_pk.hip
@@ -144,3 +144,9 @@
 
 }
 }
+
+#ifdef CLICA_LP_TRACE
+extern "C" int clica_debug_lp_trace(unsigned long long* buf) {
+  return (int)hipMemcpyToSymbol(HIP_SYMBOL(clica::lp::g_lp_trace), &buf, sizeof(buf));
+}
+#endif
diff --git a/cl_ica_amd/csrc/nn_search.hip b/cl_ica_amd/csrc/nn_search.hip
--- a/cl_ica_amd/csrc/nn_search.hip
+++ b/cl_ica_amd/csrc/nn_search.hip
@@ -44,7 +44,8 @@
   const int64_t je = min(n_tab, jb + (int64_t)chunk);
   Stager<NP> st;
   if (jb < je) {
-    st.load(tab, ldt, jb, (int)min((int64_t)TS, je - jb), q.n);
+    st.init(tab, ldt, jb, q.n);
+    st.load((int)min((int64_t)TS, je - jb));
     st.store(tiles[0]);
   }
   __syncthreads();
@@ -52,7 +53,7 @@
   for (int64_t j0 = jb; j0 < je; j0 += TS, cur ^= 1) {
     const int cnt = (int)min((int64_t)TS, je - j0);
     const bool more = j0 + TS < je;
-    if (more) st.load(tab, ldt, j0 + TS, (int)min((int64_t)TS, je - j0 - TS), q.n);
+    if (more) st.load((int)min((int64_t)TS, je - j0 - TS));
     const float* tile = tiles[cur] + pq * RPP * NP;
     const int cq = min(RPP, max(0, cnt - pq * RPP));
     const int row0 = (int)j0 + pq * RPP;
```

Result: faster. 2854, median of 6 (+1.5%).
